# limanling/clip-event

Measured on AMD Instinct MI355X. Metric: image-text pairs/sec/GPU, ViT-B/32 224px x 77-tok, global-batch contrastive, higher is better.
Workload: dtype bf16; 1 GPU; ViT-B/32 224px x 77-tok, bf16 operands, per-GPU batch 256, K=1, InfoNCE only, full train step (fwd+bwd+clip_grad_norm+Adam), random-init weights; global_batch=256, parallelism=dp1, captions=SOT + U[8,75] random ids + EOT, zero-padded to 77 (SURVEY 8(d) c2), text_rows=live tokens SOT..EOT only: 54.8% of B*77 rows (identical results, see DESIGN.md), fresh_captions_every_step=True, alignment=False, cu_hog=0, nt_pgrid=256, full=False

## Files before the change

clip_event_amd/csrc/gemm.hip:

```cpp
#include <stdlib.h>

#include <map>
#include <mutex>
#include <type_traits>

#include "common.hpp"
#include "nt_plan.hpp"
#include "tn_plan.hpp"
#include "../../include/clip_event_hip.h"

#ifndef CE_DIAG_TN3
#define CE_DIAG_TN3 0
#endif

namespace {

constexpr int NT_BM = 128, NT_BN = 128, NT_BK = 64;
constexpr int NT_STAGE_BYTES = (NT_BM + NT_BN) * NT_BK * 2;
constexpr int NT_LDS_BYTES = 2 * NT_STAGE_BYTES;

#include "gemm_common.hpp"

template <int EPI>
__global__ __launch_bounds__(256, 2) void gemm_nt_kernel(NTArgs p) {
// ... 1224 lines not shown
        const int cur = mt & 1;
        if (mt + 1 < nmt) issue_loads(mt + 1);
        const char* st = smem + cur * TN_STAGE_BYTES;
#pragma unroll
        for (int s = 0; s < 4; ++s) {
            bf16x8 pf[2], qf[2];
#pragma unroll
            for (int t = 0; t < 2; ++t) {
                pf[t] = tr_frag(st, tp_base + s * 16 * TN_ROW + t * 64);
                qf[t] = tr_frag(st, tq_base + s * 16 * TN_ROW + t * 64);
            }
#pragma unroll
            for (int nt = 0; nt < 2; ++nt)
#pragma unroll
                for (int kt = 0; kt < 2; ++kt)
                    acc[nt][kt] = __builtin_amdgcn_mfma_f32_32x32x16_bf16(pf[nt], qf[kt], acc[nt][kt], 0, 0, 0);
        }
        if (mt + 1 < nmt) write_stage(cur ^ 1);
        __syncthreads();
    }

    const int ek = k0 + wk * 64 + (lane & 31);
    const int en = n0 + wn * 64 + 4 * (lane >> 5);
#pragma unroll
    for (int nt = 0; nt < 2; ++nt)
#pragma unroll
        for (int kt = 0; kt < 2; ++kt) {
            const int k = ek + kt * 32;
            if (k >= p.Kk) continue;
#pragma unroll
            for (int r = 0; r < 16; ++r) {
                const int n = en + nt * 32 + (r & 3) + 8 * (r >> 2);
                if (n < p.Nn) atomicAdd(p.out + (long)n * p.ldo + k, acc[nt][kt][r]);
            }
        }
}

constexpr int T2_TILE_BYTES = TN_BM * 256;
constexpr int T2_STAGE_BYTES = 2 * T2_TILE_BYTES;
constexpr int T2_LDS_BYTES = 2 * T2_STAGE_BYTES;

__device__ __forceinline__ bf16x8 tr_frag2(const char* p) {
    typedef __attribute__((address_space(3))) s16x4 lds_s16x4;
    s16x4 lo = __builtin_amdgcn_ds_read_tr16_b64_v4i16((lds_s16x4*)(p));
    s16x4 hi = __builtin_amdgcn_ds_read_tr16_b64_v4i16((lds_s16x4*)(p + 4 * 256));
    typedef __attribute__((ext_vector_type(8))) short s16x8;
    s16x8 v = {lo[0], lo[1], lo[2], lo[3], hi[0], hi[1], hi[2], hi[3]};
    return __builtin_bit_cast(bf16x8, v);
}

struct TNGroup {
    int count, splits, m_per_split, M, depth;
    int overwrite = 0;
    int tile_end[CE_TN_MAX_GROUP];
    TNArgs prob[CE_TN_MAX_GROUP];
};

__global__ __launch_bounds__(256, 2) void gemm_tn2_kernel(TNGroup grp) {
    extern __shared__ __attribute__((aligned(16))) char smem[];
    const int tid = threadIdx.x;
    const int lane = tid & 63;
    const int wave = __builtin_amdgcn_readfirstlane(tid >> 6);
    const int wn = wave >> 1, wk = wave & 1;

    const int m_tiles = (grp.M + TN_BM - 1) / TN_BM;
    const int mps = grp.m_per_split / TN_BM;
    const int s_r = lane >> 4;
    const int s_chunk = (lane & 15) ^ (s_r << 2);
    const int g = lane >> 4, li = lane & 15;
    const int t_row = 8 * (g >> 1) + (li >> 2);
    const int t_sw = (li >> 2) << 2;
    const int t_cb = 2 * (g & 1) + ((li & 3) >> 1);
    int offP[2], offQ[2];
#pragma unroll
    for (int t = 0; t < 2; ++t) {
        offP[t] = t_row * 256 + (((wn * 8 + t * 4 + t_cb) ^ t_sw) << 4) + (li & 1) * 8;
        offQ[t] = T2_TILE_BYTES + t_row * 256 + (((wk * 8 + t * 4 + t_cb) ^ t_sw) << 4) + (li & 1) * 8;
    }

    {
        const int lb = xcd_remap(blockIdx.x, gridDim.x);
        int tile = lb / grp.splits;
        const int mt0 = (lb - tile * grp.splits) * mps;
        const int mt1 = min(m_tiles, mt0 + mps);
        if (mt0 >= mt1) return;
        int pi = 0;
        while (pi + 1 < grp.count && tile >= grp.tile_end[pi]) ++pi;
        if (pi > 0) tile -= grp.tile_end[pi - 1];
        const TNArgs& p = grp.prob[pi];
        int tn, tk;
        {
            constexpr int BNB = 4, BKB = 4;
            const int br = tile / (BNB * p.tiles_k);
            const int r0 = br * BNB, rows_b = min(BNB, p.tiles_n - r0);
            const int t1 = tile - br * BNB * p.tiles_k;
            const int bc = t1 / (rows_b * BKB);
            const int c0 = bc * BKB, cols_b = min(BKB, p.tiles_k - c0);
            const int t2 = t1 - bc * rows_b * BKB;
            tn = r0 + t2 / cols_b;
            tk = c0 + t2 % cols_b;
        }
        const int n0 = tn * TN_BN, k0 = tk * TN_BK;
        const int ms = mt0 * TN_BM;
        const int rows = min(grp.M, mt1 * TN_BM) - ms;
        const long ldp = p.ldp, ldq = p.ldq;

        const u32x4 rP = make_rsrc_words(p.P + (long)ms * ldp, (uint32_t)((long)rows * ldp * 2));
        const u32x4 rQ = make_rsrc_words(p.Q + (long)ms * ldq, (uint32_t)((long)rows * ldq * 2));
        uint32_t vP[4], vQ[4];
// ... 17 lines not shown
        };

        f32x16 acc[2][2];
#pragma unroll
        for (int r = 0; r < 16; ++r) {
            acc[0][0][r] = 0.f; acc[0][1][r] = 0.f; acc[1][0][r] = 0.f; acc[1][1][r] = 0.f;
        }

        const int nmt = mt1 - mt0;
        stage(0, 0);
        asm volatile("s_waitcnt vmcnt(0)" ::: "memory");
        __syncthreads();
        for (int mt = 0; mt < nmt; ++mt) {
            const int cur = mt & 1;
            if (mt + 1 < nmt) stage(cur ^ 1, mt + 1);
            const char* st = smem + cur * T2_STAGE_BYTES;
#pragma unroll
            for (int s = 0; s < 4; ++s) {
                bf16x8 pf[2], qf[2];
#pragma unroll
                for (int t = 0; t < 2; ++t) {
                    pf[t] = tr_frag2(st + offP[t] + s * 16 * 256);
                    qf[t] = tr_frag2(st + offQ[t] + s * 16 * 256);
                }
#pragma unroll
                for (int nt = 0; nt < 2; ++nt)
#pragma unroll
                    for (int kt = 0; kt < 2; ++kt)
                        acc[nt][kt] = __builtin_amdgcn_mfma_f32_32x32x16_bf16(pf[nt], qf[kt], acc[nt][kt], 0, 0, 0);
            }
            asm volatile("s_waitcnt vmcnt(0)" ::: "memory");
            __syncthreads();
        }

        const int ek = k0 + wk * 64 + (lane & 31);
        const int en = n0 + wn * 64 + 4 * (lane >> 5);
        constexpr bool sole = false;
#pragma unroll
        for (int nt = 0; nt < 2; ++nt)
#pragma unroll
            for (int kt = 0; kt < 2; ++kt) {
                const int k = ek + kt * 32;
                if (k >= p.Kk) continue;
#pragma unroll
                for (int r = 0; r < 16; ++r) {
                    const int n = en + nt * 32 + (r & 3) + 8 * (r >> 2);
                    if (n < p.Nn) {
                        float* o = p.out + (long)n * p.ldo + k;
                        if (sole) *o += acc[nt][kt][r];
                        else atomicAdd(o, acc[nt][kt][r]);
                    }
                }
            }
    }
}

template <int T3_ROWS, int T3_STAGES>
__global__ __launch_bounds__(1024, 4) void gemm_tn3_kernel(TNGroup grp) {
    constexpr int T3_IMG_BYTES = T3_ROWS * 256;
    constexpr int T3_STAGE_BYTES = 4 * T3_IMG_BYTES;
    constexpr int KSTEPS = T3_ROWS / 16;
    constexpr int DPW = T3_ROWS / 16;
    extern __shared__ __attribute__((aligned(16))) char smem[];
    const int tid = threadIdx.x;
    const int lane = tid & 63;
    const int wave = __builtin_amdgcn_readfirstlane(tid >> 6);
    const int wn = wave >> 2, wk = wave & 3;

    const int m_tiles = (grp.M + TN_BM - 1) / TN_BM;
    const int mps = grp.m_per_split / TN_BM;
    const int s_r = lane >> 4;
    const int s_chunk = (lane & 15) ^ (s_r << 2);
    const int g = lane >> 4, li = lane & 15;
    const int t_row = 8 * (g >> 1) + (li >> 2);
    const int t_sw = (li >> 2) << 2;
    const int t_cb = 2 * (g & 1) + ((li & 3) >> 1);
    int offP[2], offQ[2];
#pragma unroll
    for (int t = 0; t < 2; ++t) {
        offP[t] = (wn >> 1) * T3_IMG_BYTES + t_row * 256 + ((((wn & 1) * 8 + t * 4 + t_cb) ^ t_sw) << 4) + (li & 1) * 8;
        offQ[t] = (2 + (wk >> 1)) * T3_IMG_BYTES + t_row * 256 + ((((wk & 1) * 8 + t * 4 + t_cb) ^ t_sw) << 4) + (li & 1) * 8;
    }

    const int lb = xcd_remap(blockIdx.x, gridDim.x);
    int tile = lb / grp.splits;
    const int mt0 = (lb - tile * grp.splits) * mps;
    const int mt1 = min(m_tiles, mt0 + mps);
    if (mt0 >= mt1) return;
    int pi = 0;
    while (pi + 1 < grp.count && tile >= grp.tile_end[pi]) ++pi;
    if (pi > 0) tile -= grp.tile_end[pi - 1];
    const TNArgs& p = grp.prob[pi];
    int tn, tk;
    {
        constexpr int BNB = 2, BKB = 2;
        const int br = tile / (BNB * p.tiles_k);
        const int r0 = br * BNB, rows_b = min(BNB, p.tiles_n - r0);
        const int t1 = tile - br * BNB * p.tiles_k;
        const int bc = t1 / (rows_b * BKB);
        const int c0 = bc * BKB, cols_b = min(BKB, p.tiles_k - c0);
        const int t2 = t1 - bc * rows_b * BKB;
        tn = r0 + t2 / cols_b;
        tk = c0 + t2 % cols_b;
    }
    const int n0 = tn * 256, k0 = tk * 256;
    const int ms = mt0 * TN_BM;
// ... 24 lines not shown
    for (int r = 0; r < 16; ++r) {
        acc[0][0][r] = 0.f; acc[0][1][r] = 0.f; acc[1][0][r] = 0.f; acc[1][1][r] = 0.f;
    }

    const int nst = (rows + T3_ROWS - 1) / T3_ROWS;
    const int D = min(grp.depth, T3_STAGES - 1);
    stage(0, 0);
    if (nst > 1 && D > 1) stage(1, 1);
    if (nst > 2 && D > 2) stage(2, 2);
    int slot = 0;
    for (int i = 0; i < nst; ++i) {
        const int later = min(nst - 1 - i, D - 1);
        if (later == 2) asm volatile("s_waitcnt vmcnt(%0)" ::"n"(2 * DPW) : "memory");
        else if (later == 1) asm volatile("s_waitcnt vmcnt(%0)" ::"n"(DPW) : "memory");
        else asm volatile("s_waitcnt vmcnt(0)" ::: "memory");
        __builtin_amdgcn_s_barrier();
        if (i + D < nst) {
            int sl = slot + D;
            if (sl >= T3_STAGES) sl -= T3_STAGES;
            stage(sl, i + D);
        }
        const char* st = smem + slot * T3_STAGE_BYTES;
        slot = slot + 1 == T3_STAGES ? 0 : slot + 1;
#pragma unroll
        for (int s = 0; s < KSTEPS; ++s) {
            bf16x8 pf[2], qf[2];
#pragma unroll
            for (int t = 0; t < 2; ++t) {
                pf[t] = tr_frag2(st + offP[t] + s * 16 * 256);
                qf[t] = tr_frag2(st + offQ[t] + s * 16 * 256);
            }
#pragma unroll
            for (int nt = 0; nt < 2; ++nt)
#pragma unroll
                for (int kt = 0; kt < 2; ++kt)
                    acc[nt][kt] = __builtin_amdgcn_mfma_f32_32x32x16_bf16(pf[nt], qf[kt], acc[nt][kt], 0, 0, 0);
        }
    }

    const int ek = k0 + wk * 64 + (lane & 31);
    const int en = n0 + wn * 64 + 4 * (lane >> 5);
#pragma unroll
    for (int nt = 0; nt < 2; ++nt)
#pragma unroll
        for (int kt = 0; kt < 2; ++kt) {
            const int k = ek + kt * 32;
#pragma unroll
            for (int r = 0; r < 16; ++r) {
                const int n = en + nt * 32 + (r & 3) + 8 * (r >> 2);
                if (grp.overwrite) __builtin_nontemporal_store(acc[nt][kt][r], p.out + (long)n * p.ldo + k);
                else atomicAdd(p.out + (long)n * p.ldo + k, acc[nt][kt][r]);
            }
        }
}

template <int T3_ROWS, int T3_STAGES>
__global__ __launch_bounds__(768, 3) void gemm_tn3lw_kernel(TNGroup grp) {
    constexpr int T3_IMG_BYTES = T3_ROWS * 256;
    constexpr int T3_STAGE_BYTES = 4 * T3_IMG_BYTES;
    constexpr int KSTEPS = T3_ROWS / 16;
    constexpr int DPL = T3_ROWS / 4;
    extern __shared__ __attribute__((aligned(16))) char smem[];
    const int tid = threadIdx.x;
    const int lane = tid & 63;
    const int wave = __builtin_amdgcn_readfirstlane(tid >> 6);
    const int wn = (wave >> 2) & 1, wk = wave & 3;

    const int m_tiles = (grp.M + TN_BM - 1) / TN_BM;
    const int mps = grp.m_per_split / TN_BM;
    const int s_r = lane >> 4;
    const int s_chunk = (lane & 15) ^ (s_r << 2);
    const int g = lane >> 4, li = lane & 15;
    const int t_row = 8 * (g >> 1) + (li >> 2);
    const int t_sw = (li >> 2) << 2;
    const int t_cb = 2 * (g & 1) + ((li & 3) >> 1);
    int offP[4], offQ[2];
#pragma unroll
    for (int t = 0; t < 4; ++t)
        offP[t] = wn * T3_IMG_BYTES + t_row * 256 + (((t * 4 + t_cb) ^ t_sw) << 4) + (li & 1) * 8;
#pragma unroll
    for (int t = 0; t < 2; ++t)
        offQ[t] = (2 + (wk >> 1)) * T3_IMG_BYTES + t_row * 256 + ((((wk & 1) * 8 + t * 4 + t_cb) ^ t_sw) << 4) + (li & 1) * 8;

    const int lb = xcd_remap(blockIdx.x, gridDim.x);
    int tile = lb / grp.splits;
    const int mt0 = (lb - tile * grp.splits) * mps;
    const int mt1 = min(m_tiles, mt0 + mps);
    if (mt0 >= mt1) return;
    int pi = 0;
    while (pi + 1 < grp.count && tile >= grp.tile_end[pi]) ++pi;
    if (pi > 0) tile -= grp.tile_end[pi - 1];
    const TNArgs& p = grp.prob[pi];
    int tn, tk;
    {
        constexpr int BNB = 2, BKB = 2;
        const int br = tile / (BNB * p.tiles_k);
        const int r0 = br * BNB, rows_b = min(BNB, p.tiles_n - r0);
        const int t1 = tile - br * BNB * p.tiles_k;
        const int bc = t1 / (rows_b * BKB);
        const int c0 = bc * BKB, cols_b = min(BKB, p.tiles_k - c0);
        const int t2 = t1 - bc * rows_b * BKB;
        tn = r0 + t2 / cols_b;
        tk = c0 + t2 % cols_b;
    }
    const int n0 = tn * 256, k0 = tk * 256;
    const int ms = mt0 * TN_BM;
// ... 21 lines not shown
#endif
                dma16_bounds(rsrc, d + j * 1024, vo0 + j * vstep + mb);
            }
        };
        stage(0, 0);
        if (nst > 1 && D > 1) stage(1, 1);
        if (nst > 2 && D > 2) stage(2, 2);
        int slot = 0;
        for (int i = 0; i < nst; ++i) {
            const int later = min(nst - 1 - i, D - 1);
            if (later == 2) asm volatile("s_waitcnt vmcnt(%0)" ::"n"(2 * DPL) : "memory");
            else if (later == 1) asm volatile("s_waitcnt vmcnt(%0)" ::"n"(DPL) : "memory");
            else asm volatile("s_waitcnt vmcnt(0)" ::: "memory");
            __builtin_amdgcn_s_barrier();
            if (i + D < nst) {
                int sl = slot + D;
                if (sl >= T3_STAGES) sl -= T3_STAGES;
                stage(sl, i + D);
            }
            slot = slot + 1 == T3_STAGES ? 0 : slot + 1;
        }
        return;
    }

    f32x16 acc[4][2];
#pragma unroll
    for (int nt = 0; nt < 4; ++nt)
#pragma unroll
        for (int r = 0; r < 16; ++r) {
            acc[nt][0][r] = 0.f; acc[nt][1][r] = 0.f;
        }
    int slot = 0;
    for (int i = 0; i < nst; ++i) {
        __builtin_amdgcn_s_barrier();
        const char* st = smem + slot * T3_STAGE_BYTES;
        slot = slot + 1 == T3_STAGES ? 0 : slot + 1;
#pragma unroll
        for (int s = 0; s < KSTEPS; ++s) {
            bf16x8 qf[2];
#pragma unroll
            for (int t = 0; t < 2; ++t) qf[t] = tr_frag2(st + offQ[t] + s * 16 * 256);
#pragma unroll
            for (int nt = 0; nt < 4; ++nt) {
                const bf16x8 pf = tr_frag2(st + offP[nt] + s * 16 * 256);
#pragma unroll
                for (int kt = 0; kt < 2; ++kt)
                    acc[nt][kt] = __builtin_amdgcn_mfma_f32_32x32x16_bf16(pf, qf[kt], acc[nt][kt], 0, 0, 0);
            }
        }
    }

    const int ek = k0 + wk * 64 + (lane & 31);
    const int en = n0 + wn * 128 + 4 * (lane >> 5);
#pragma unroll
    for (int nt = 0; nt < 4; ++nt)
#pragma unroll
        for (int kt = 0; kt < 2; ++kt) {
            const int k = ek + kt * 32;
#pragma unroll
            for (int r = 0; r < 16; ++r) {
                const int n = en + nt * 32 + (r & 3) + 8 * (r >> 2);
#if CE_DIAG_TN3 == 1
                if (acc[nt][kt][r] == 12345.678f)
#endif
                if (grp.overwrite) __builtin_nontemporal_store(acc[nt][kt][r], p.out + (long)n * p.ldo + k);
                else atomicAdd(p.out + (long)n * p.ldo + k, acc[nt][kt][r]);
            }
        }
}

__global__ void probe_mfma16_kernel(const bf16x8* a, const bf16x8* b, f32x4* out) {
    f32x4 c = {0.f, 0.f, 0.f, 0.f};
    c = __builtin_amdgcn_mfma_f32_16x16x32_bf16(a[threadIdx.x], b[threadIdx.x], c, 0, 0, 0);
    out[threadIdx.x] = c;
}
__global__ void probe_mfma32_kernel(const bf16x8* a, const bf16x8* b, f32x16* out) {
    f32x16 c;
#pragma unroll
    for (int r = 0; r < 16; ++r) c[r] = 0.f;
    c = __builtin_amdgcn_mfma_f32_32x32x16_bf16(a[threadIdx.x], b[threadIdx.x], c, 0, 0, 0);
    out[threadIdx.x] = c;
}
__global__ void probe_tr16_kernel(const uint16_t* image, int n_elems, const int* byte_off, s16x4* out) {
    extern __shared__ __attribute__((aligned(16))) char smem[];
    uint16_t* l = reinterpret_cast<uint16_t*>(smem);
    for (int i = threadIdx.x; i < n_elems; i += 64) l[i] = image[i];
    __syncthreads();
    typedef __attribute__((address_space(3))) s16x4 lds_s16x4;
    out[threadIdx.x] = __builtin_amdgcn_ds_read_tr16_b64_v4i16((lds_s16x4*)(smem + byte_off[threadIdx.x]));
}

static_assert(NT_PLAN_LDS[NT_NT128] == NT_LDS_BYTES && NT_PLAN_LDS[NT_NT256x2] == N2H_LDS_BYTES && NT_PLAN_LDS[NT_NT256x4] == N2_LDS_BYTES &&
              NT_PLAN_LDS[NT_NT32] == N3_LDS_BYTES && NT_PLAN_LDS[NT_NT160_RING] == N4_LDS_BYTES && NT_PLAN_LDS[NT_LW] == N4_LDS_BYTES &&
              NT_PLAN_LDS[NT_PERSIST] == N4P_LDS_BYTES && NT_PLAN_LDS[NT_SKINNY] == SK_LDS_BYTES &&
              NT_PLAN_BLOCK[NT_LW] == 64 * (8 + N4_LOADERS), "nt_plan.hpp is out of step with the kernels");

int env_int(const char* name, int otherwise) {
    const char* e = getenv(name);
    return e ? atoi(e) : otherwise;
}
NTKnobs knobs_from_env() {
    NTKnobs k;
    k.cus = env_int("CE_GEMM_CUS", 256);
    k.dynamic = env_int("CE_NT_DYNAMIC", 0);
    k.env_chunk = env_int("CE_NT_CHUNK", 0);
    k.env_pgrid = env_int("CE_NT_PGRID", 0);
// ... 175 lines not shown
        case CE_EPI_BIAS_F32:
            CE_CHECK_ARG(bias, "ce_gemm_nt: bias epilogue without bias");
            return launch_nt<CE_EPI_BIAS_F32, 0>(a, s);
        case CE_EPI_BIAS_RESID_F32:
            CE_CHECK_ARG(bias && resid && ldr >= N && ldr % 4 == 0, "ce_gemm_nt: residual epilogue needs bias+resid");
            return launch_nt<CE_EPI_BIAS_RESID_F32, 0>(a, s);
        case CE_EPI_BIAS_RESID_F16:
            CE_CHECK_ARG(bias && resid && ldr >= N && ldr % 8 == 0 && ldo % 8 == 0, "ce_gemm_nt: fp16 residual epilogue needs bias+resid, ldr/ldo multiples of 8");
            return launch_nt<CE_EPI_BIAS_RESID_F16, 0>(a, s);
        case CE_EPI_BIAS_GELU:
            CE_CHECK_ARG(bias && out2 && ldo2 >= N && ldo2 % 4 == 0, "ce_gemm_nt: gelu epilogue needs bias+out2");
            return launch_nt<CE_EPI_BIAS_GELU, 0>(a, s);
        case CE_EPI_BIAS_QGELU_BF16:
            CE_CHECK_ARG(bias, "ce_gemm_nt: QuickGELU epilogue without bias");
            return launch_nt<CE_EPI_BIAS_QGELU_BF16, 0>(a, s);
        case CE_EPI_GELUGRAD_BF16:
            CE_CHECK_ARG(aux && ldaux >= N && ldaux % 4 == 0, "ce_gemm_nt: gelu-grad epilogue needs aux");
            return launch_nt<CE_EPI_GELUGRAD_BF16, 0>(a, s);
        default: CE_CHECK_ARG(false, "ce_gemm_nt: unknown epilogue %d", epilogue);
    }
    return 0;
}

extern "C" int ce_gemm_tn(const void* P, long ldp, const void* Q, long ldq, int M, int Nn, int Kk, float* out,
                          long ldo, int splits, void* stream) {
    return ce_gemm_tn_bias(P, ldp, Q, ldq, M, Nn, Kk, out, ldo, nullptr, splits, stream);
}

extern "C" int ce_gemm_tn_bias(const void* P, long ldp, const void* Q, long ldq, int M, int Nn, int Kk, float* out,
                               long ldo, float* bias_grad, int splits, void* stream) {
    const void* Ps[1] = {P};
    const void* Qs[1] = {Q};
    float* outs[1] = {out};
    int rc = ce_gemm_tn_grouped(1, Ps, &ldp, Qs, &ldq, M, &Nn, &Kk, outs, &ldo, splits, stream);
    if (rc != 0) return rc;
    if (bias_grad) return ce_colsum_bf16(P, ldp, bias_grad, M, Nn, stream);
    return 0;
}

extern "C" int ce_gemm_tn_grouped(int count, const void* const* P, const long* ldp, const void* const* Q,
                                  const long* ldq, int M, const int* Nn, const int* Kk, float* const* out,
                                  const long* ldo, int splits, void* stream) {
    return ce_gemm_tn_grouped_ex(count, P, ldp, Q, ldq, M, Nn, Kk, out, ldo, splits, 0, stream);
}

static_assert(TN_PLAN_BM == TN_BM && TN_PLAN_LDS_V1 == TN_LDS_BYTES && TN_PLAN_LDS_128 == T2_LDS_BYTES &&
              tn_plan_lds_256(48, 3) == 3 * 48 * 1024 && tn_plan_lds_256(32, 4) == 4 * 32 * 1024 && TN_PLAN_BLOCK[TN_V1] == 256 &&
              TN_PLAN_BLOCK[TN_V2] == 256 && TN_PLAN_BLOCK[TN_V3] == 1024 && TN_PLAN_BLOCK[TN_V3LW] == 768,
              "tn_plan.hpp is out of step with the kernels");

extern "C" int ce_gemm_tn_grouped_ex(int count, const void* const* P, const long* ldp, const void* const* Q,
                                     const long* ldq, int M, const int* Nn, const int* Kk, float* const* out,
                                     const long* ldo, int splits, int overwrite, void* stream) {
    CE_CHECK_ARG(count >= 1 && count <= CE_TN_MAX_GROUP && M > 0, "ce_gemm_tn_grouped: 1..%d problems, M > 0", CE_TN_MAX_GROUP);
    hipStream_t s = (hipStream_t)stream;
    TNGroup g;
    g.count = count;
    g.M = M;
    double flops = 0.0, bytes = 0.0;
    long ldmax = 0;
    for (int i = 0; i < count; ++i) {
        CE_CHECK_ARG(Nn[i] > 0 && Kk[i] > 0, "ce_gemm_tn: empty problem");
        CE_CHECK_ARG(Nn[i] % 8 == 0 && Kk[i] % 8 == 0 && ldp[i] % 8 == 0 && ldq[i] % 8 == 0,
                     "ce_gemm_tn: Nn,Kk,ldp,ldq must be multiples of 8");
        CE_CHECK_ARG(ldp[i] >= Nn[i] && ldq[i] >= Kk[i] && ldo[i] >= Kk[i], "ce_gemm_tn: leading dimension smaller than the row");
        TNArgs& a = g.prob[i];
        a.P = (const bf16_t*)P[i]; a.ldp = ldp[i]; a.Q = (const bf16_t*)Q[i]; a.ldq = ldq[i];
        a.out = out[i]; a.ldo = ldo[i]; a.M = M; a.Nn = Nn[i]; a.Kk = Kk[i];
        flops += 2.0 * M * Nn[i] * Kk[i];
        bytes += 2.0 * ((double)M * Nn[i] + (double)M * Kk[i]) + 8.0 * Nn[i] * Kk[i];
        if (ldp[i] > ldmax) ldmax = ldp[i];
        if (ldq[i] > ldmax) ldmax = ldq[i];
    }
    CE_CHECK_ARG((long)M * ldmax * 2 < (1L << 32), "ce_gemm_tn: operand exceeds 4 GiB");

    const TNPlan p = tn_plan(M, count, Nn, Kk, splits, overwrite != 0, tn_process_knobs());
    g.splits = p.splits; g.m_per_split = p.m_per_split; g.depth = p.depth; g.overwrite = p.kernel_overwrites;
    for (int i = 0; i < CE_TN_MAX_GROUP; ++i) g.tile_end[i] = p.tile_end[i];
    for (int i = 0; i < count; ++i) {
        TNArgs& a = g.prob[i];
        a.tiles_n = p.tiles_n[i]; a.tiles_k = p.tiles_k[i]; a.splits = p.splits; a.m_per_split = p.m_per_split;
    }
    if (p.zero_fill_first)
        for (int i = 0; i < count; ++i)
            if (hipMemset2DAsync(out[i], (size_t)ldo[i] * 4, 0, (size_t)Kk[i] * 4, (size_t)Nn[i], s) != hipSuccess) {
                ce_set_error("ce_gemm_tn_grouped: zero-fill of output %d failed", i);
                return -5;
            }

    constexpr auto key = [](int form, int rows) { return 64 * form + rows; };
#define CE_TN_CASE(FORM, ROWS, ...)                                                      \
    case key(FORM, ROWS): {                                                              \
        CeProfScope prof(p.prof_class, flops, bytes, s);                                 \
        launch_kernel<__VA_ARGS__>(p.workgroups, p.block, p.lds_bytes, g, s);            \
    } break
    switch (key(p.form, p.rows)) {
        case key(TN_V1, 64):
            for (int i = 0; i < count; ++i) {
                const TNArgs& a = g.prob[i];
                CeProfScope prof(p.prof_class, 2.0 * M * a.Nn * a.Kk, 0.0, s);
                launch_kernel<gemm_tn_kernel>(a.tiles_n * a.tiles_k * a.splits, p.block, p.lds_bytes, a, s);
            }
            break;
        CE_TN_CASE(TN_V2, 64, gemm_tn2_kernel);
        CE_TN_CASE(TN_V3, 32, gemm_tn3_kernel<32, 4>);
        CE_TN_CASE(TN_V3, 48, gemm_tn3_kernel<48, 3>);
        CE_TN_CASE(TN_V3LW, 48, gemm_tn3lw_kernel<48, 3>);
        CE_TN_CASE(TN_V3LW, 32, gemm_tn3lw_kernel<32, 4>);
        default: CE_CHECK_ARG(false, "ce_gemm_tn_grouped: no kernel of form %d with %d-row stages", (int)p.form, p.rows);
    }
#undef CE_TN_CASE
    CE_LAUNCH_CHECK();
    return 0;
}

extern "C" int ce_gemm_tn_plan(int count, const int* Nn, const int* Kk, int M, int splits, int overwrite, const ce_tn_knobs* knobs,
                               ce_tn_plan* out) {
    CE_CHECK_ARG(out && Nn && Kk && count >= 1 && count <= CE_TN_MAX_GROUP && M > 0,
                 "ce_gemm_tn_plan: 1..%d problems, M > 0 and a result struct", CE_TN_MAX_GROUP);
    for (int i = 0; i < count; ++i) CE_CHECK_ARG(Nn[i] > 0 && Kk[i] > 0, "ce_gemm_tn_plan: empty problem %d", i);
    *out = tn_plan(M, count, Nn, Kk, splits, overwrite != 0, knobs ? TNKnobs(*knobs) : tn_process_knobs());
    return 0;
}

extern "C" int ce_probe_mfma(int shape, const void* a_frags, const void* b_frags, float* out, void* stream) {
    if (shape == 16)
        hipLaunchKernelGGL(probe_mfma16_kernel, dim3(1), dim3(64), 0, (hipStream_t)stream, (const bf16x8*)a_frags,
                           (const bf16x8*)b_frags, (f32x4*)out);
    else if (shape == 32)
        hipLaunchKernelGGL(probe_mfma32_kernel, dim3(1), dim3(64), 0, (hipStream_t)stream, (const bf16x8*)a_frags,
                           (const bf16x8*)b_frags, (f32x16*)out);
    else
        CE_CHECK_ARG(false, "ce_probe_mfma: shape must be 16 or 32");
    CE_LAUNCH_CHECK();
    return 0;
}

extern "C" int ce_probe_tr16(const void* image, int n_elems, const int* byte_off, void* out, void* stream) {
    CE_CHECK_ARG(n_elems > 0 && n_elems <= 16384, "ce_probe_tr16: image must hold 1..16384 elements");
    hipLaunchKernelGGL(probe_tr16_kernel, dim3(1), dim3(64), n_elems * 2, (hipStream_t)stream, (const uint16_t*)image,
                       n_elems, byte_off, (s16x4*)out);
    CE_LAUNCH_CHECK();
    return 0;
}
```

clip_event_amd/csrc/optim.hip:

```cpp
#include <stdlib.h>

#include "common.hpp"
#include "../../include/clip_event_hip.h"

#ifndef CE_ADAM_NT
#define CE_ADAM_NT 2
#endif
#if CE_ADAM_NT >= 1
#define CE_ADAM_ST(val, ptr) __builtin_nontemporal_store(val, ptr)
#else
#define CE_ADAM_ST(val, ptr) (*(ptr) = (val))
#endif
#if CE_ADAM_NT >= 2
#define CE_ADAM_LD(ptr) __builtin_nontemporal_load(ptr)
#else
#define CE_ADAM_LD(ptr) (*(ptr))
#endif

namespace {

__global__ __launch_bounds__(256) void sumsq_kernel(const float* __restrict__ g, long n, float* __restrict__ out) {
    __shared__ float red[4];
    float s = 0.f;
    const long stride = gridDim.x * 1024L;
// ... 261 lines not shown
}
template <class Rule>
__device__ __forceinline__ void store_state(float* const (&st)[2], long at, const f32x4 (&sv)[kSlots<Rule>]) {
#pragma unroll
    for (int k = 0; k < Rule::NS; ++k) CE_ADAM_ST(sv[k], reinterpret_cast<f32x4*>(st[k] + at));
}
__device__ __forceinline__ u32x2 pack_bf4(const f32x4& v) { return u32x2{pack_bf2(v[0], v[1]), pack_bf2(v[2], v[3])}; }

template <class Rule, bool EMA>
__global__ __launch_bounds__(256) void optim_flat_kernel(float* __restrict__ p, const float* __restrict__ g, float* __restrict__ s0,
                                                         float* __restrict__ s1, bf16_t* __restrict__ p16, long n,
                                                         typename Rule::Args a, float* __restrict__ ema, float ema_rate) {
    const Rule rule(a, 0);
    float* const st[2] = {s0, s1};
    const long stride = gridDim.x * 2048L;
    for (long i0 = blockIdx.x * 2048L + threadIdx.x * 4; i0 < n; i0 += stride) {
        const long i1 = i0 + 1024;
        if (i1 + 3 < n) {
            f32x4 pv[2], gv[2], sv[2][kSlots<Rule>] = {}, ev[2] = {};
#pragma unroll
            for (int u = 0; u < 2; ++u) load_chunk<Rule, EMA>(p, g, st, ema, u ? i1 : i0, pv[u], gv[u], sv[u], ev[u]);
#pragma unroll
            for (int u = 0; u < 2; ++u) {
                const long i = u ? i1 : i0;
                elem4(rule, pv[u], gv[u], sv[u]);
                CE_ADAM_ST(pv[u], reinterpret_cast<f32x4*>(p + i));
                if (p16) *reinterpret_cast<u32x2*>(p16 + i) = pack_bf4(pv[u]);
                store_state<Rule>(st, i, sv[u]);
                update_ema<EMA>(ema, i, ev[u], pv[u], ema_rate);
            }
        } else {
            for (int u = 0; u < 2; ++u) {
                const long ib = u ? i1 : i0;
                for (long k = ib; k < n && k < ib + 4; ++k) {
                    float pk = p[k], sk[kSlots<Rule>] = {};
#pragma unroll
                    for (int q = 0; q < Rule::NS; ++q) sk[q] = st[q][k];
                    rule.elem(pk, g[k], sk);
                    p[k] = pk;
#pragma unroll
                    for (int q = 0; q < Rule::NS; ++q) st[q][k] = sk[q];
                    if (p16) p16[k] = f2bf(pk);
                    if constexpr (EMA) {
                        float ek = ema[k];
                        ema_elem(ek, pk, ema_rate);
                        ema[k] = ek;
                    }
                }
            }
        }
    }
}

__global__ __launch_bounds__(256) void zero_segments_kernel(float* __restrict__ base, const long* __restrict__ table) {
    const long lo = table[2 * blockIdx.x], hi = table[2 * blockIdx.x + 1];
    for (long i = lo + threadIdx.x * 4; i < hi; i += 1024)
        __builtin_nontemporal_store(f32x4{0.f, 0.f, 0.f, 0.f}, reinterpret_cast<f32x4*>(base + i));
}

struct tile_at {
    ce_transpose_job job;
    int r0, c0;
};
__device__ __forceinline__ tile_at find_tile(const ce_transpose_job* __restrict__ jobs, int njobs) {
    int j = 0;
    const int b = blockIdx.x;
    while (j + 1 < njobs && b >= jobs[j + 1].tile_start) ++j;
    const ce_transpose_job job = jobs[j];
    const int t = b - job.tile_start;
    const int tiles_c = (job.cols + 63) / 64;
    return {job, (t / tiles_c) * 64, (t % tiles_c) * 64};
}

template <bool NT>
__device__ __forceinline__ void store_tile_transposed(const bf16_t (&tile)[64][66], const tile_at& t) {
    bf16_t* dst = reinterpret_cast<bf16_t*>(t.job.dst);
#pragma unroll
    for (int k = 0; k < 2; ++k) {
        const int idx = threadIdx.x + k * 256;
        const int c = idx >> 3, ch = idx & 7;
        if (t.c0 + c < t.job.cols && t.r0 + ch * 8 < t.job.rows) {
            uint32_t w[4];
#pragma unroll
            for (int e = 0; e < 4; ++e)
                w[e] = (uint32_t)tile[ch * 8 + 2 * e][c] | ((uint32_t)tile[ch * 8 + 2 * e + 1][c] << 16);
            const u32x4 v = {w[0], w[1], w[2], w[3]};
            u32x4* out = reinterpret_cast<u32x4*>(dst + (long)(t.c0 + c) * t.job.rows + t.r0 + ch * 8);
            if (NT) __builtin_nontemporal_store(v, out);
            else *out = v;
        }
    }
}

__global__ __launch_bounds__(256) void multi_transpose_kernel(const ce_transpose_job* __restrict__ jobs, int njobs) {
    __shared__ bf16_t tile[64][66];
    const tile_at t = find_tile(jobs, njobs);
    const ce_transpose_job& job = t.job;
    const int r0 = t.r0, c0 = t.c0;
    const bf16_t* src = reinterpret_cast<const bf16_t*>(job.src);
    bf16_t* dst = reinterpret_cast<bf16_t*>(job.dst);
    const bool wide = (job.rows % 8 == 0) && (job.cols % 8 == 0) &&
                      ((reinterpret_cast<size_t>(src) | reinterpret_cast<size_t>(dst)) % 16 == 0);
    if (wide) {
#pragma unroll
        for (int k = 0; k < 2; ++k) {
            const int idx = threadIdx.x + k * 256;
            const int r = idx >> 3, ch = idx & 7;
// ... 142 lines not shown
    const long blocks = (n + 2047) / 2048;
    return (unsigned)(blocks > cap ? cap : blocks);
}
template <class Rule>
void launch_flat(float* p, const float* g, float* s0, float* s1, void* p_bf16, long n, const typename Rule::Args& a, void* stream,
                 float* ema = nullptr, float ema_rate = 0.f) {
    if (ema)
        hipLaunchKernelGGL((optim_flat_kernel<Rule, true>), dim3(flat_blocks(n)), dim3(256), 0, (hipStream_t)stream, p, g, s0, s1,
                           (bf16_t*)p_bf16, n, a, ema, ema_rate);
    else
        hipLaunchKernelGGL((optim_flat_kernel<Rule, false>), dim3(flat_blocks(n)), dim3(256), 0, (hipStream_t)stream, p, g, s0, s1,
                           (bf16_t*)p_bf16, n, a, ema, 0.f);
}

template <class Rule>
void launch_tiles(float* p, const float* g, float* s0, float* s1, void* p_bf16, const ce_transpose_job* jobs_device, int njobs,
                  int total_tiles, const long* segments_device, int nsegments, const typename Rule::Args& a, void* stream,
                  float* ema = nullptr, float ema_rate = 0.f) {
    const hipStream_t s = (hipStream_t)stream;
    if (jobs_device && njobs > 0 && total_tiles > 0) {
        if (ema)
            hipLaunchKernelGGL((optim_tiles_kernel<Rule, true>), dim3((unsigned)total_tiles), dim3(256), 0, s, p, g, s0, s1,
                               (bf16_t*)p_bf16, jobs_device, njobs, a, ema, ema_rate);
        else
            hipLaunchKernelGGL((optim_tiles_kernel<Rule, false>), dim3((unsigned)total_tiles), dim3(256), 0, s, p, g, s0, s1,
                               (bf16_t*)p_bf16, jobs_device, njobs, a, ema, 0.f);
    }
    if (segments_device && nsegments > 0) {
        if (ema)
            hipLaunchKernelGGL((optim_segments_kernel<Rule, true>), dim3((unsigned)nsegments), dim3(256), 0, s, p, g, s0, s1,
                               (bf16_t*)p_bf16, segments_device, a, ema, ema_rate);
        else
            hipLaunchKernelGGL((optim_segments_kernel<Rule, false>), dim3((unsigned)nsegments), dim3(256), 0, s, p, g, s0, s1,
                               (bf16_t*)p_bf16, segments_device, a, ema, 0.f);
    }
}

int ema_check(const char* who, const float* ema, float ema_rate) {
    CE_CHECK_ARG(ema, "%s: ema is NULL", who);
    CE_CHECK_ARG(ema_rate > 0.f && ema_rate <= 1.f, "%s: ema_rate %g is outside (0, 1]", who, (double)ema_rate);
    return 0;
}

}

extern "C" int ce_multi_transpose_bf16(const ce_transpose_job* jobs_device, int njobs, int total_tiles, void* stream) {
    CE_CHECK_ARG(jobs_device && njobs > 0 && total_tiles > 0, "ce_multi_transpose_bf16: empty");
    hipLaunchKernelGGL(multi_transpose_kernel, dim3(total_tiles), dim3(256), 0, (hipStream_t)stream, jobs_device, njobs);
    CE_LAUNCH_CHECK();
    return 0;
}

extern "C" int ce_zero_segments(float* base, const long* table_device, int nchunks, void* stream) {
    CE_CHECK_ARG(base && table_device && nchunks > 0, "ce_zero_segments: empty");
    hipLaunchKernelGGL(zero_segments_kernel, dim3(nchunks), dim3(256), 0, (hipStream_t)stream, base, table_device);
    CE_LAUNCH_CHECK();
    return 0;
}

extern "C" int ce_sumsq(const float* g, long n, float* out, void* stream) {
    CE_CHECK_ARG(n > 0, "ce_sumsq: empty");
    long blocks = (n + 1023) / 1024;
    if (blocks > 2048) blocks = 2048;
    hipLaunchKernelGGL(sumsq_kernel, dim3((unsigned)blocks), dim3(256), 0, (hipStream_t)stream, g, n, out);
    CE_LAUNCH_CHECK();
    return 0;
}


namespace {

int adam_step(const char* who, float* p, const float* g, float* m, float* v, void* p_bf16, long n, const float* sumsq, float max_norm,
              float lr, float beta1, float beta2, float eps, float weight_decay, int step, float* ema, float ema_rate, void* stream) {
    CE_CHECK_ARG(n > 0 && step >= 1, "%s: need n>0 and step>=1", who);
    launch_flat<AdamRule>(p, g, m, v, p_bf16, n, adam_args(sumsq, max_norm, lr, beta1, beta2, eps, weight_decay, step), stream, ema,
                          ema_rate);
    CE_LAUNCH_CHECK();
    return 0;
}

int adam_step_tiles(const char* who, float* p, const float* g, float* m, float* v, void* p_bf16, const ce_transpose_job* jobs_device,
                    int njobs, int total_tiles, const long* segments_device, int nsegments, const float* sumsq, float max_norm, float lr,
                    float beta1, float beta2, float eps, float weight_decay, int step, float* ema, float ema_rate, void* stream) {
    CE_CHECK_ARG(p && g && m && v && p_bf16 && step >= 1, "%s: null buffer or step < 1", who);
    CE_CHECK_ARG((jobs_device && njobs > 0 && total_tiles > 0) || (segments_device && nsegments > 0), "%s: nothing to update", who);
    launch_tiles<AdamRule>(p, g, m, v, p_bf16, jobs_device, njobs, total_tiles, segments_device, nsegments,
                           adam_args(sumsq, max_norm, lr, beta1, beta2, eps, weight_decay, step), stream, ema, ema_rate);
    CE_LAUNCH_CHECK();
    return 0;
}

int sgd_step(const char* who, float* p, const float* g, float* buf, void* p_bf16, long n, const float* sumsq, float max_norm, float lr,
             float momentum, float dampening, float weight_decay, int nesterov, int first_step, float* ema, float ema_rate,
             void* stream) {
    CE_CHECK_ARG(n > 0, "%s: need n>0", who);
    if (int rc = sgd_check(who, buf, momentum, dampening, nesterov)) return rc;
    CE_CHECK_ARG(p && g, "%s: null buffer", who);
    const sgd_args a = {sumsq, max_norm, lr, momentum, 1.0f - dampening, weight_decay, first_step != 0, nesterov != 0};
    if (momentum > 0.f) launch_flat<SgdRule<true>>(p, g, buf, nullptr, p_bf16, n, a, stream, ema, ema_rate);
    else launch_flat<SgdRule<false>>(p, g, nullptr, nullptr, p_bf16, n, a, stream, ema, ema_rate);
    CE_LAUNCH_CHECK();
    return 0;
}

int sgd_step_tiles(const char* who, float* p, const float* g, float* buf, void* p_bf16, const ce_transpose_job* jobs_device, int njobs,
                   int total_tiles, const long* segments_device, int nsegments, const float* sumsq, float max_norm, float lr,
                   float momentum, float dampening, float weight_decay, int nesterov, int first_step, float* ema, float ema_rate,
                   void* stream) {
    if (int rc = sgd_check(who, buf, momentum, dampening, nesterov)) return rc;
    CE_CHECK_ARG((jobs_device && njobs > 0 && total_tiles > 0) || (segments_device && nsegments > 0), "%s: nothing to update", who);
    CE_CHECK_ARG(p && g && p_bf16, "%s: null buffer", who);
    const sgd_args a = {sumsq, max_norm, lr, momentum, 1.0f - dampening, weight_decay, first_step != 0, nesterov != 0};
    if (momentum > 0.f)
        launch_tiles<SgdRule<true>>(p, g, buf, nullptr, p_bf16, jobs_device, njobs, total_tiles, segments_device, nsegments, a, stream,
                                    ema, ema_rate);
    else
// ... 103 lines not shown
                                float* ema, float ema_rate, void* stream) {
    if (int rc = ema_check("ce_adam_step_ema", ema, ema_rate)) return rc;
    return adam_step("ce_adam_step_ema", p, g, m, v, p_bf16, n, sumsq, max_norm, lr, beta1, beta2, eps, weight_decay, step, ema,
                     ema_rate, stream);
}

extern "C" int ce_adam_step_tiles(float* p, const float* g, float* m, float* v, void* p_bf16, const ce_transpose_job* jobs_device,
                                  int njobs, int total_tiles, const long* segments_device, int nsegments, const float* sumsq,
                                  float max_norm, float lr, float beta1, float beta2, float eps, float weight_decay, int step,
                                  void* stream) {
    return adam_step_tiles("ce_adam_step_tiles", p, g, m, v, p_bf16, jobs_device, njobs, total_tiles, segments_device, nsegments, sumsq,
                           max_norm, lr, beta1, beta2, eps, weight_decay, step, nullptr, 0.f, stream);
}
extern "C" int ce_adam_step_tiles_ema(float* p, const float* g, float* m, float* v, void* p_bf16, const ce_transpose_job* jobs_device,
                                      int njobs, int total_tiles, const long* segments_device, int nsegments, const float* sumsq,
                                      float max_norm, float lr, float beta1, float beta2, float eps, float weight_decay, int step,
                                      float* ema, float ema_rate, void* stream) {
    if (int rc = ema_check("ce_adam_step_tiles_ema", ema, ema_rate)) return rc;
    return adam_step_tiles("ce_adam_step_tiles_ema", p, g, m, v, p_bf16, jobs_device, njobs, total_tiles, segments_device, nsegments,
                           sumsq, max_norm, lr, beta1, beta2, eps, weight_decay, step, ema, ema_rate, stream);
}

extern "C" int ce_sgd_step(float* p, const float* g, float* buf, void* p_bf16, long n, const float* sumsq, float max_norm, float lr,
                           float momentum, float dampening, float weight_decay, int nesterov, int first_step, void* stream) {
    return sgd_step("ce_sgd_step", p, g, buf, p_bf16, n, sumsq, max_norm, lr, momentum, dampening, weight_decay, nesterov, first_step,
                    nullptr, 0.f, stream);
}
extern "C" int ce_sgd_step_ema(float* p, const float* g, float* buf, void* p_bf16, long n, const float* sumsq, float max_norm, float lr,
                               float momentum, float dampening, float weight_decay, int nesterov, int first_step, float* ema,
                               float ema_rate, void* stream) {
    if (int rc = ema_check("ce_sgd_step_ema", ema, ema_rate)) return rc;
    return sgd_step("ce_sgd_step_ema", p, g, buf, p_bf16, n, sumsq, max_norm, lr, momentum, dampening, weight_decay, nesterov,
                    first_step, ema, ema_rate, stream);
}

extern "C" int ce_sgd_step_tiles(float* p, const float* g, float* buf, void* p_bf16, const ce_transpose_job* jobs_device, int njobs,
                                 int total_tiles, const long* segments_device, int nsegments, const float* sumsq, float max_norm,
                                 float lr, float momentum, float dampening, float weight_decay, int nesterov, int first_step,
                                 void* stream) {
    return sgd_step_tiles("ce_sgd_step_tiles", p, g, buf, p_bf16, jobs_device, njobs, total_tiles, segments_device, nsegments, sumsq,
                          max_norm, lr, momentum, dampening, weight_decay, nesterov, first_step, nullptr, 0.f, stream);
}
extern "C" int ce_sgd_step_tiles_ema(float* p, const float* g, float* buf, void* p_bf16, const ce_transpose_job* jobs_device, int njobs,
                                     int total_tiles, const long* segments_device, int nsegments, const float* sumsq, float max_norm,
                                     float lr, float momentum, float dampening, float weight_decay, int nesterov, int first_step,
                                     float* ema, float ema_rate, void* stream) {
    if (int rc = ema_check("ce_sgd_step_tiles_ema", ema, ema_rate)) return rc;
    return sgd_step_tiles("ce_sgd_step_tiles_ema", p, g, buf, p_bf16, jobs_device, njobs, total_tiles, segments_device, nsegments, sumsq,
                          max_norm, lr, momentum, dampening, weight_decay, nesterov, first_step, ema, ema_rate, stream);
}

extern "C" int ce_sumsq_segments(const float* g, const long* table_device, int nchunks, float* out, void* stream) {
    CE_CHECK_ARG(g && table_device && out && nchunks > 0, "ce_sumsq_segments: empty");
    hipLaunchKernelGGL(sumsq_segments_kernel, dim3((unsigned)nchunks), dim3(256), 0, (hipStream_t)stream, g, table_device, out);
    CE_LAUNCH_CHECK();
    return 0;
}

extern "C" int ce_adam_step_groups(float* p, const float* g, float* m, float* v, void* p_bf16, const ce_transpose_job* jobs_device,
                                   int njobs, int total_tiles, const long* segments_device, int nsegments, const int* segment_group,
                                   const float* sumsq, float max_norm, const ce_optim_group* groups, int ngroups, float beta1,
                                   float beta2, float eps, int step, void* stream) {
    return adam_step_groups("ce_adam_step_groups", p, g, m, v, p_bf16, jobs_device, njobs, total_tiles, segments_device, nsegments,
                            segment_group, sumsq, max_norm, groups, ngroups, beta1, beta2, eps, step, nullptr, 0.f, stream);
}
extern "C" int ce_adam_step_groups_ema(float* p, const float* g, float* m, float* v, void* p_bf16, const ce_transpose_job* jobs_device,
                                       int njobs, int total_tiles, const long* segments_device, int nsegments, const int* segment_group,
                                       const float* sumsq, float max_norm, const ce_optim_group* groups, int ngroups, float beta1,
                                       float beta2, float eps, int step, float* ema, float ema_rate, void* stream) {
    if (int rc = ema_check("ce_adam_step_groups_ema", ema, ema_rate)) return rc;
    return adam_step_groups("ce_adam_step_groups_ema", p, g, m, v, p_bf16, jobs_device, njobs, total_tiles, segments_device, nsegments,
                            segment_group, sumsq, max_norm, groups, ngroups, beta1, beta2, eps, step, ema, ema_rate, stream);
}

extern "C" int ce_sgd_step_groups(float* p, const float* g, float* buf, void* p_bf16, const ce_transpose_job* jobs_device, int njobs,
                                  int total_tiles, const long* segments_device, int nsegments, const int* segment_group,
                                  const float* sumsq, float max_norm, const ce_optim_group* groups, int ngroups, float momentum,
                                  float dampening, int nesterov, int first_step, void* stream) {
    return sgd_step_groups("ce_sgd_step_groups", p, g, buf, p_bf16, jobs_device, njobs, total_tiles, segments_device, nsegments,
                           segment_group, sumsq, max_norm, groups, ngroups, momentum, dampening, nesterov, first_step, nullptr, 0.f,
                           stream);
}
extern "C" int ce_sgd_step_groups_ema(float* p, const float* g, float* buf, void* p_bf16, const ce_transpose_job* jobs_device, int njobs,
                                      int total_tiles, const long* segments_device, int nsegments, const int* segment_group,
                                      const float* sumsq, float max_norm, const ce_optim_group* groups, int ngroups, float momentum,
                                      float dampening, int nesterov, int first_step, float* ema, float ema_rate, void* stream) {
    if (int rc = ema_check("ce_sgd_step_groups_ema", ema, ema_rate)) return rc;
    return sgd_step_groups("ce_sgd_step_groups_ema", p, g, buf, p_bf16, jobs_device, njobs, total_tiles, segments_device, nsegments,
                           segment_group, sumsq, max_norm, groups, ngroups, momentum, dampening, nesterov, first_step, ema, ema_rate,
                           stream);
}

extern "C" int ce_lion_step(float* p, const float* g, float* m, void* p_bf16, long n, const float* sumsq, float max_norm, float lr,
                            float beta1, float beta2, float weight_decay, void* stream) {
    return lion_step("ce_lion_step", p, g, m, p_bf16, n, sumsq, max_norm, lr, beta1, beta2, weight_decay, nullptr, 0.f, stream);
}
extern "C" int ce_lion_step_ema(float* p, const float* g, float* m, void* p_bf16, long n, const float* sumsq, float max_norm, float lr,
                                float beta1, float beta2, float weight_decay, float* ema, float ema_rate, void* stream) {
    if (int rc = ema_check("ce_lion_step_ema", ema, ema_rate)) return rc;
    return lion_step("ce_lion_step_ema", p, g, m, p_bf16, n, sumsq, max_norm, lr, beta1, beta2, weight_decay, ema, ema_rate, stream);
}

extern "C" int ce_lion_step_tiles(float* p, const float* g, float* m, void* p_bf16, const ce_transpose_job* jobs_device, int njobs,
                                  int total_tiles, const long* segments_device, int nsegments, const float* sumsq, float max_norm,
                                  float lr, float beta1, float beta2, float weight_decay, void* stream) {
    return lion_step_tiles("ce_lion_step_tiles", p, g, m, p_bf16, jobs_device, njobs, total_tiles, segments_device, nsegments, sumsq,
// ... 36 lines not shown
```

clip_event_amd/csrc/tn_plan.cpp:

```cpp
#include "tn_plan.hpp"

#include <stdlib.h>

namespace {

inline int div_up(long a, long b) { return (int)((a + b - 1) / b); }

inline void set_splits(TNPlan& p, int M, int splits) {
    const int m_tiles = div_up(M, TN_PLAN_BM);
    if (splits > m_tiles) splits = m_tiles;
    if (splits < 1) splits = 1;
    p.m_per_split = div_up(m_tiles, splits) * TN_PLAN_BM;
    p.splits = div_up(M, p.m_per_split);
}

inline int env_int(const char* name, int otherwise) {
    const char* e = getenv(name);
    return e ? atoi(e) : otherwise;
}

}

TNKnobs tn_knobs_from_env() {
    TNKnobs k;
// ... 29 lines not shown
        p.lds_bytes = p.form == TN_V1 ? TN_PLAN_LDS_V1 : TN_PLAN_LDS_128;
        set_splits(p, M, splits_arg > 0 ? splits_arg : 512 / tiles);
        p.prof_class = CE_PROF_GEMM_TN2;
    } else {
        auto cost = [&](int sp) {
            const long wgs = (long)tiles * sp;
            const long rounds = (wgs + 255) / 256;
            const long tail = wgs - (rounds - 1) * 256;
            return rounds * (div_up(m_tiles, sp) * 1.7 + 3.0) + tail * (sp == 1 ? 0.105 : 0.20);
        };
        int sp = 1;
        if (splits_arg > 0) sp = splits_arg;
        else if (knobs.force_splits > 0) sp = knobs.force_splits;
        else {
            double best = cost(1);
            for (int c = 2; c <= 16 && c <= m_tiles && (long)tiles * c <= 256; ++c)
                if (cost(c) < best) { best = cost(c); sp = c; }
        }
        set_splits(p, M, sp);
        p.rows = knobs.rows == 32 ? 32 : 48;
        p.stages = p.rows == 48 ? 3 : 4;
        p.form = knobs.loader_waves ? TN_V3LW : TN_V3;
        p.lds_bytes = tn_plan_lds_256(p.rows, p.stages);
        p.kernel_overwrites = overwrite && p.splits == 1;
        p.prof_class = CE_PROF_GEMM_TN;
    }
    p.zero_fill_first = overwrite && !p.kernel_overwrites;
    p.block = TN_PLAN_BLOCK[p.form];
    p.workgroups = tiles * p.splits;
    return p;
}

int tn_group_cuts(int n_blocks, int width, int M, long extra_tiles, int force_group, int* sizes_out) {
    const int n = n_blocks;
    if (force_group > TN_GROUP_MAX_BLOCKS) force_group = TN_GROUP_MAX_BLOCKS;
    const long t = 12 * tn_problem_tiles(M, width, width);
    const long slots = tn_round_slots(M, width, width);
    long cost[TN_CUT_MAX_BLOCKS + 1];
    int take[TN_CUT_MAX_BLOCKS + 1];
    cost[0] = 0;
    for (int k = 1; k <= n; ++k) {
        cost[k] = -1;
        for (int g = 1; g <= TN_GROUP_MAX_BLOCKS && g <= k; ++g) {
            if (force_group >= 1 && g != force_group && g != k) continue;
            const long tiles = g * t + (k == n ? extra_tiles : 0);
            const long c = cost[k - g] + (tiles + slots - 1) / slots * 1000 + 1;
            if (cost[k] < 0 || c < cost[k]) { cost[k] = c; take[k] = g; }
        }
    }
    int groups = 0;
    for (int k = n; k > 0; k -= take[k]) sizes_out[groups++] = take[k];
    return groups;
}
```

clip_event_amd/csrc/tn_plan.hpp:

```cpp
#pragma once
#include "../../include/clip_event_hip.h"

enum TNForm {
    TN_V1 = 0,
    TN_V2 = 1,
    TN_V3 = 2,
    TN_V3LW = 3
};

constexpr int TN_PLAN_BLOCK[4] = {256, 256, 1024, 768};
constexpr int TN_PLAN_LDS_128 = 65536;
constexpr int TN_PLAN_LDS_V1 = 81920;
constexpr int tn_plan_lds_256(int rows, int stages) { return stages * rows * 1024; }

constexpr int TN_PLAN_BM = 64;
constexpr int TN_PLAN_MIN_M_256 = 2048;

constexpr bool tn_tiles_256(int M, int Nn, int Kk) { return M >= TN_PLAN_MIN_M_256 && Nn % 256 == 0 && Kk % 256 == 0; }
constexpr long tn_problem_tiles(int M, int Nn, int Kk) {
    return tn_tiles_256(M, Nn, Kk) ? (long)(Nn / 256) * (Kk / 256) : (long)((Nn + 127) / 128) * ((Kk + 127) / 128);
}
constexpr int tn_round_slots(int M, int Nn, int Kk) { return tn_tiles_256(M, Nn, Kk) ? 256 : 512; }

struct TNKnobs : ce_tn_knobs {
    constexpr TNKnobs() : ce_tn_knobs{3, 0, 3, 48, 1} {}
    constexpr TNKnobs(const ce_tn_knobs& k) : ce_tn_knobs(k) {}
};
TNKnobs tn_knobs_from_env();
const TNKnobs& tn_process_knobs();

using TNPlan = ce_tn_plan;

TNPlan tn_plan(int M, int count, const int* Nn, const int* Kk, int splits_arg, bool overwrite, const TNKnobs& knobs);

constexpr int TN_CUT_MAX_BLOCKS = 64;
constexpr int TN_GROUP_MAX_BLOCKS = 8;

int tn_group_cuts(int n_blocks, int width, int M, long extra_tiles, int force_group, int* sizes_out);
```

clip_event_amd/csrc/tower.cpp:

```cpp
#include <hip/hip_runtime.h>
#include <stdlib.h>

#include <map>
#include <mutex>

#include "common.hpp"
#include "tn_plan.hpp"
#include "../../include/clip_event_hip.h"

namespace {

constexpr int WG_MAX_BLOCKS = TN_GROUP_MAX_BLOCKS;
constexpr int WG_SETS = WG_MAX_BLOCKS + 1;
constexpr int LNP_RING = 8;

struct Carver {
    char* base;
    size_t off = 0;
    explicit Carver(void* b) : base(reinterpret_cast<char*>(b)) {}
    template <typename T>
    T* take(size_t n) {
        off = (off + 255) & ~size_t(255);
        T* p = base ? reinterpret_cast<T*>(base + off) : nullptr;
        off += n * sizeof(T);
        return p;
    }
};

struct BlockStash {
    void* x_mid;
    void* x_out;
    bf16_t *h1, *qkv, *o, *h2, *a, *g;
    float *mean1, *rstd1, *mean2, *rstd2, *lse;
};

struct Layout {
    static constexpr int MAX_LAYERS = 64;
    BlockStash blk[MAX_LAYERS];
    bf16_t *dxb[WG_SETS], *dxb2[WG_SETS], *da[WG_SETS], *dqkv[WG_SETS];
    bf16_t *dh, *d_o;
    uint8_t* q8;
    float* q8s;
    float *xs_in, *xs_mid, *dxs_mid, *means, *rstds;
    bf16_t *os, *h2s, *as, *gs, *dxbs, *dxb2s, *das, *dhs, *dos;
    float* lnp[LNP_RING][2];
    size_t bytes;
};

void carve(const ce_tower_desc* d, int batch, size_t rows, void* ws, Layout& L) {
    Carver c(ws);
    const size_t M = rows, w = d->width;
    const size_t esz = d->stream16 ? 2 : 4;
    for (int l = 0; l < d->layers; ++l) {
        BlockStash& s = L.blk[l];
        s.x_mid = c.take<char>(M * w * esz);
        s.x_out = (l + 1 < d->layers) ? c.take<char>(M * w * esz) : nullptr;
        s.h1 = c.take<bf16_t>(M * w);
        s.qkv = c.take<bf16_t>(M * 3 * w);
        s.o = c.take<bf16_t>(M * w);
        s.h2 = c.take<bf16_t>(M * w);
        s.a = c.take<bf16_t>(M * 4 * w);
        s.g = c.take<bf16_t>(M * 4 * w);
        s.mean1 = c.take<float>(M);
        s.rstd1 = c.take<float>(M);
        s.mean2 = c.take<float>(M);
        s.rstd2 = c.take<float>(M);
        s.lse = c.take<float>((size_t)batch * d->heads * d->tokens);
    }
    for (int q = 0; q < WG_SETS; ++q) {
        L.dxb[q] = c.take<bf16_t>(M * w);
        L.dxb2[q] = c.take<bf16_t>(M * w);
        L.da[q] = c.take<bf16_t>(M * 4 * w);
        L.dqkv[q] = c.take<bf16_t>(M * 3 * w);
    }
    L.dh = c.take<bf16_t>(M * w);
    L.d_o = c.take<bf16_t>(M * w);
    L.q8 = d->fp8 ? c.take<uint8_t>(M * 4 * w) : nullptr;
    L.q8s = d->fp8 ? c.take<float>(M) : nullptr;
    const size_t Bn = (size_t)batch;
    L.xs_in = c.take<float>(Bn * w); L.xs_mid = c.take<float>(Bn * w); L.dxs_mid = c.take<float>(Bn * w);
    L.means = c.take<float>(Bn); L.rstds = c.take<float>(Bn);
    L.os = c.take<bf16_t>(Bn * w); L.h2s = c.take<bf16_t>(Bn * w); L.as = c.take<bf16_t>(Bn * 4 * w); L.gs = c.take<bf16_t>(Bn * 4 * w);
    L.dxbs = c.take<bf16_t>(Bn * w); L.dxb2s = c.take<bf16_t>(Bn * w); L.das = c.take<bf16_t>(Bn * 4 * w);
    L.dhs = c.take<bf16_t>(Bn * w); L.dos = c.take<bf16_t>(Bn * w);
    const size_t lnp_floats = (size_t)ce_layernorm_bwd_blocks((int)M, (int)w) * 3 * w;
    for (int l = 0; l < LNP_RING; ++l) {
        L.lnp[l][0] = l < d->layers ? c.take<float>(lnp_floats) : nullptr;
        L.lnp[l][1] = l < d->layers ? c.take<float>(lnp_floats) : nullptr;
    }
    L.bytes = (c.off + 255) & ~size_t(255);
}

void carve_infer(const ce_tower_desc* d, int batch, size_t rows, void* ws, Layout& L) {
    Carver c(ws);
    const size_t M = rows, w = d->width;
    const size_t esz = d->stream16 ? 2 : 4;
    L = Layout{};
    BlockStash s{};
    s.x_mid = c.take<char>(M * w * esz);
    s.x_out = c.take<char>(M * w * esz);
    s.h1 = s.h2 = c.take<bf16_t>(M * w);
    s.qkv = c.take<bf16_t>(M * 3 * w);
    s.o = c.take<bf16_t>(M * w);
    s.a = nullptr;
    s.g = c.take<bf16_t>(M * 4 * w);
    s.mean1 = s.mean2 = c.take<float>(M);
    s.rstd1 = s.rstd2 = c.take<float>(M);
    s.lse = c.take<float>((size_t)batch * d->heads * d->tokens);
    for (int l = 0; l < d->layers; ++l) L.blk[l] = s;
    L.blk[d->layers - 1].x_out = nullptr;
    L.q8 = d->fp8 ? c.take<uint8_t>(M * 4 * w) : nullptr;
    L.q8s = d->fp8 ? c.take<float>(M) : nullptr;
    const size_t Bn = (size_t)batch;
    L.xs_in = c.take<float>(Bn * w); L.xs_mid = c.take<float>(Bn * w);
    L.means = c.take<float>(Bn); L.rstds = c.take<float>(Bn);
    L.os = c.take<bf16_t>(Bn * w); L.h2s = c.take<bf16_t>(Bn * w); L.gs = c.take<bf16_t>(Bn * 4 * w);
    L.bytes = (c.off + 255) & ~size_t(255);
}

int check_rows(const ce_tower_desc* d, int batch, int rows, const int* cu) {
    CE_CHECK_ARG(rows > 0 && (long)rows <= (long)batch * d->tokens, "tower: rows=%d outside 1..batch*tokens", rows);
    CE_CHECK_ARG(cu || rows == batch * d->tokens, "tower: a dense batch has batch*tokens rows (got %d)", rows);
    return 0;
}

int check_desc(const ce_tower_desc* d, int batch) {
    CE_CHECK_ARG(d && d->blocks, "tower: null descriptor");
    CE_CHECK_ARG(d->layers > 0 && d->layers <= Layout::MAX_LAYERS, "tower: layers=%d out of range", d->layers);
    CE_CHECK_ARG(d->width == d->heads * 64, "tower: width %d != heads %d * 64", d->width, d->heads);
    CE_CHECK_ARG(d->tokens > 0 && d->tokens <= 4096, "tower: tokens=%d unsupported (1..4096)", d->tokens);
    CE_CHECK_ARG(batch > 0, "tower: empty batch");
    CE_CHECK_ARG(d->stream16 == 0 || d->stream16 == 1, "tower: stream16=%d (0: fp32 residual stream, 1: fp16)", d->stream16);
    return 0;
}

#define TRY(call)            \
    do {                     \
        int rc__ = (call);   \
        if (rc__ != 0) return rc__; \
    } while (0)

// ... 69 lines not shown
extern "C" int ce_tower_forward(const ce_tower_desc* d, int batch, int rows, const int* cu_seqlens, const void* x0,
                                void* workspace, void* x_out, const int* sel_rows, void* stream) {
    TRY(check_desc(d, batch));
    TRY(check_rows(d, batch, rows, cu_seqlens));
    CE_CHECK_ARG(x0 && workspace && x_out, "ce_tower_forward: null buffer");
    Layout L;
    carve(d, batch, rows, workspace, L);
    return forward_run(d, batch, rows, cu_seqlens, x0, L, x_out, sel_rows, false, stream);
}

extern "C" size_t ce_tower_infer_workspace_bytes(const ce_tower_desc* d, int batch) {
    if (check_desc(d, batch) != 0) return 0;
    Layout L;
    carve_infer(d, batch, (size_t)batch * d->tokens, nullptr, L);
    return L.bytes;
}

extern "C" int ce_tower_forward_infer(const ce_tower_desc* d, int batch, int rows, const int* cu_seqlens, const void* x0,
                                      void* workspace, void* x_out, const int* sel_rows, void* stream) {
    TRY(check_desc(d, batch));
    TRY(check_rows(d, batch, rows, cu_seqlens));
    CE_CHECK_ARG(x0 && workspace && x_out, "ce_tower_forward_infer: null buffer");
    Layout L;
    carve_infer(d, batch, rows, workspace, L);
    return forward_run(d, batch, rows, cu_seqlens, x0, L, x_out, sel_rows, true, stream);
}

extern "C" int ce_tower_backward(const ce_tower_desc* d, int batch, int rows, const int* cu_seqlens, const void* x0,
                                 void* workspace, void* dx, const int* sel_rows, const float* dx_sel, void* stream) {
    return ce_tower_backward_range(d, batch, rows, cu_seqlens, x0, workspace, dx, sel_rows, dx_sel,
                                   d ? d->layers - 1 : 0, 0, stream);
}

extern "C" int ce_tower_backward_range(const ce_tower_desc* d, int batch, int rows, const int* cu_seqlens,
                                       const void* x0, void* workspace, void* dx, const int* sel_rows,
                                       const float* dx_sel, int layer_hi, int layer_lo, void* stream) {
    TRY(check_desc(d, batch));
    TRY(check_rows(d, batch, rows, cu_seqlens));
    CE_CHECK_ARG(x0 && workspace && dx, "ce_tower_backward: null buffer");
    CE_CHECK_ARG(layer_lo >= 0 && layer_lo <= layer_hi && layer_hi < d->layers, "ce_tower_backward_range: layers %d..%d outside 0..%d",
                 layer_hi, layer_lo, d->layers - 1);
    Layout L;
    carve(d, batch, rows, workspace, L);
    const int M = rows, w = d->width;
    const bool b8 = (d->fp8 & 2) != 0;
    const int ST = d->stream16 ? CE_T_F16 : CE_T_F32;
    const void* q8_of = nullptr;
    const bool lnq = b8 && w % 128 == 0 && w <= 4096;
    const float* GS = d->stream16 ? d->grad_scale : nullptr;
    CE_CHECK_ARG(!d->stream16 || GS, "ce_tower_backward: stream16 needs ce_tower_desc.grad_scale (device pointer)");
    const long esz = d->stream16 ? 2 : 4;
    const int last = d->layers - 1;
    static const int ln_fold = getenv("CE_LN_FOLD") ? atoi(getenv("CE_LN_FOLD")) : 1;
    ce_ln_fold_job fold_jobs[2 * LNP_RING];
    int n_fold = 0;
    int fold_rc = 0;
    const int ln_blocks = ce_layernorm_bwd_blocks(M, w);
    auto ln_bwd = [&](const void* dy, const void* xin, const float* mean, const float* rstd, const float* gamma, void* dxb, float* dgw, float* dgb,
                      float* dxs, void* q8, float* partial) -> int {
        if (!ln_fold)
            return ce_layernorm_bwd_q8(dy, CE_T_BF16, w, xin, ST, w, nullptr, mean, rstd, gamma, dx, ST, dx, ST, w, dxb, w, dgw, dgb, dxs, GS, M, w, q8, w,
                                       L.q8s, stream);
        fold_jobs[n_fold++] = ce_ln_fold_job{partial, dgw, dgb, dxs, ln_blocks, w};
        const int rc = ce_layernorm_bwd_partials(dy, CE_T_BF16, w, xin, ST, w, nullptr, mean, rstd, gamma, dx, ST, dx, ST, w, dxb, w, dxs ? 1 : 0, GS, M, w, q8, w,
                                                 L.q8s, partial, stream);
        if (rc == 0 && n_fold == 2 * LNP_RING) {
            fold_rc = ce_layernorm_fold(fold_jobs, n_fold, stream);
            n_fold = 0;
            return fold_rc;
        }
        return rc;
    };
    static const int force_group = getenv("CE_WGRAD_GROUP") ? atoi(getenv("CE_WGRAD_GROUP")) : 0;
    bool cut_after[Layout::MAX_LAYERS] = {};
    auto plan_cuts = [&](int hi, int lo, long extra_tiles) {
        static_assert(Layout::MAX_LAYERS <= TN_CUT_MAX_BLOCKS, "tn_group_cuts takes fewer blocks than a tower has");
        int sizes[Layout::MAX_LAYERS];
        const int groups = tn_group_cuts(hi - lo + 1, w, M, extra_tiles, force_group, sizes);
        int l = hi;
        for (int i = 0; i < groups; ++i) {
            l -= sizes[i];
            cut_after[l + 1] = true;
        }
    };
    struct Pending {
        const void* P[CE_TN_MAX_GROUP]; long ldp[CE_TN_MAX_GROUP];
        const void* Q[CE_TN_MAX_GROUP]; long ldq[CE_TN_MAX_GROUP];
        int Nn[CE_TN_MAX_GROUP], Kk[CE_TN_MAX_GROUP];
        float* out[CE_TN_MAX_GROUP]; long ldo[CE_TN_MAX_GROUP];
        int count = 0, blocks = 0;
    } pend;
    auto queue = [&](const void* P, long ldp, const void* Q, long ldq, int Nn, int Kk, float* out, long ldo) {
        const int i = pend.count++;
        pend.P[i] = P; pend.ldp[i] = ldp; pend.Q[i] = Q; pend.ldq[i] = ldq;
        pend.Nn[i] = Nn; pend.Kk[i] = Kk; pend.out[i] = out; pend.ldo[i] = ldo;
    };
    auto flush = [&]() -> int {
        if (pend.count == 0) return 0;
        const int rc = ce_gemm_tn_grouped_ex(pend.count, pend.P, pend.ldp, pend.Q, pend.ldq, M, pend.Nn, pend.Kk, pend.out,
                                             pend.ldo, 0, d->wgrad_overwrite, stream);
        pend.count = 0;
        pend.blocks = 0;
        return rc;
    };
    int top = layer_hi;
    if (layer_hi < last) {
    } else if (sel_rows) {
        CE_CHECK_ARG(dx_sel, "ce_tower_backward: pruned mode needs dx_sel");
        const int l = top, Bn = batch, q = l % WG_SETS;
        const ce_block_params& p = d->blocks[l];
        BlockStash& s = L.blk[l];
        const void* x_in = (l == 0) ? x0 : L.blk[l - 1].x_out;
        TRY(ce_cast_bf16(dx_sel, L.dxbs, (long)Bn * w, stream));
        TRY(linear(b8, L, q8_of, L.dxbs, w, p.wt_proj, p.wt8_proj, p.st8_proj, Bn, 4 * w, w, CE_EPI_GELUGRAD_BF16, nullptr, nullptr, 0, L.das, 4 * w, nullptr,
                       0, L.as, 4 * w, stream));
        TRY(ce_colsum_bf16(L.dxbs, w, p.g_b_proj, Bn, w, stream));
        TRY(linear(b8, L, q8_of, L.das, 4 * w, p.wt_fc, p.wt8_fc, p.st8_fc, Bn, w, 4 * w, CE_EPI_BF16, nullptr, nullptr, 0, L.dhs, w, nullptr, 0,
                       nullptr, 0, stream));
        TRY(ce_colsum_bf16(L.das, 4 * w, p.g_b_fc, Bn, 4 * w, stream));
        TRY(ce_layernorm_bwd_t(L.dhs, CE_T_BF16, w, L.xs_mid, ST, w, nullptr, L.means, L.rstds, p.ln2_w, dx_sel, CE_T_F32, L.dxs_mid,
                               ST, w, L.dxb2s, w, p.g_ln2_w, p.g_ln2_b, p.g_b_out, GS, Bn, w, stream));
        TRY(linear(b8, L, q8_of, L.dxb2s, w, p.wt_out, p.wt8_out, p.st8_out, Bn, w, w, CE_EPI_BF16, nullptr, nullptr, 0, L.dos, w, nullptr, 0, nullptr, 0,
                       stream));
        TRY(ce_scatter_rows_zero(L.dos, w * 2L, L.d_o, w * 2L, sel_rows, Bn, M, w * 2, stream));
        TRY(ce_attention_bwd(s.qkv, 3 * w, s.o, w, L.d_o, w, s.lse, L.dqkv[q], 3 * w, p.g_b_qkv, cu_seqlens, batch, d->tokens, d->heads,
                             d->causal, stream));
        {
            const void* P[3] = {L.dxbs, L.das, L.dxb2s};
            const long ldp[3] = {w, 4L * w, w};
            const void* Q[3] = {L.gs, L.h2s, L.os};
            const long ldq[3] = {4L * w, w, w};
            const int Nn[3] = {w, 4 * w, w};
            const int Kk[3] = {4 * w, w, w};
            float* out[3] = {p.g_w_proj, p.g_w_fc, p.g_w_out};
            const long ldo[3] = {4L * w, w, w};
            TRY(ce_gemm_tn_grouped_ex(3, P, ldp, Q, ldq, Bn, Nn, Kk, out, ldo, 0, d->wgrad_overwrite, stream));
        }
        queue(L.dqkv[q], 3L * w, s.h1, w, 3 * w, w, p.g_w_qkv, w);
        TRY(linear(b8, L, q8_of, L.dqkv[q], 3 * w, p.wt_qkv, p.wt8_qkv, p.st8_qkv, M, w, 3 * w, CE_EPI_BF16, nullptr, nullptr, 0, L.dh, w, nullptr, 0,
                       nullptr, 0, stream));
        TRY(ce_scatter_rows_zero(L.dxs_mid, w * esz, dx, w * esz, sel_rows, Bn, M, (int)(w * esz), stream));
        TRY(ce_layernorm_bwd_t(L.dh, CE_T_BF16, w, x_in, ST, w, nullptr, s.mean1, s.rstd1, p.ln1_w, dx, ST, dx, ST, w,
                               L.dxb[(l + WG_SETS - 1) % WG_SETS], w, p.g_ln1_w, p.g_ln1_b,
                               (l > 0) ? d->blocks[l - 1].g_b_proj : nullptr, GS, M, w, stream));
        top = l - 1;
    } else {
        if (d->stream16) TRY(ce_cast_scaled(dx, ST, L.dxb[top % WG_SETS], CE_T_BF16, GS, 1, (long)M * w, stream));
        else TRY(ce_cast_bf16(reinterpret_cast<const float*>(dx), L.dxb[top % WG_SETS], (long)M * w, stream));
    }
    plan_cuts(top, layer_lo, pend.count > 0 ? 3 * tn_problem_tiles(M, w, w) : 0);
    for (int l = top; l >= layer_lo; --l) {
        const ce_block_params& p = d->blocks[l];
        BlockStash& s = L.blk[l];
        const int q = l % WG_SETS;
        bf16_t *dxb_a = L.dxb[q], *dxb_b = L.dxb2[q], *da = L.da[q], *dqkv = L.dqkv[q];
        const void* x_in = (l == 0) ? x0 : L.blk[l - 1].x_out;
        TRY(linear(b8, L, q8_of, dxb_a, w, p.wt_proj, p.wt8_proj, p.st8_proj, M, 4 * w, w, CE_EPI_GELUGRAD_BF16, nullptr, nullptr, 0, da, 4 * w, p.g_b_fc,
                       4 * w, s.a, 4 * w, stream));
        if (l == last) TRY(ce_colsum_bf16(dxb_a, w, p.g_b_proj, M, w, stream));
        TRY(linear(b8, L, q8_of, da, 4 * w, p.wt_fc, p.wt8_fc, p.st8_fc, M, w, 4 * w, CE_EPI_BF16, nullptr, nullptr, 0, L.dh, w, nullptr, 0,
                       nullptr, 0, stream));
        TRY(ln_bwd(L.dh, s.x_mid, s.mean2, s.rstd2, p.ln2_w, dxb_b, p.g_ln2_w, p.g_ln2_b, p.g_b_out, lnq ? L.q8 : nullptr, L.lnp[l % LNP_RING][1]));
        if (lnq) q8_of = dxb_b;
        TRY(linear(b8, L, q8_of, dxb_b, w, p.wt_out, p.wt8_out, p.st8_out, M, w, w, CE_EPI_BF16, nullptr, nullptr, 0, L.d_o, w, nullptr, 0, nullptr, 0,
                       stream));
        TRY(ce_attention_bwd(s.qkv, 3 * w, s.o, w, L.d_o, w, s.lse, dqkv, 3 * w, p.g_b_qkv, cu_seqlens, batch, d->tokens, d->heads,
                             d->causal, stream));
        queue(dxb_a, w, s.g, 4L * w, w, 4 * w, p.g_w_proj, 4L * w);
        queue(da, 4L * w, s.h2, w, 4 * w, w, p.g_w_fc, w);
        queue(dxb_b, w, s.o, w, w, w, p.g_w_out, w);
        queue(dqkv, 3L * w, s.h1, w, 3 * w, w, p.g_w_qkv, w);
        ++pend.blocks;
        if (cut_after[l] || pend.count + 4 > CE_TN_MAX_GROUP) TRY(flush());
        TRY(linear(b8, L, q8_of, dqkv, 3 * w, p.wt_qkv, p.wt8_qkv, p.st8_qkv, M, w, 3 * w, CE_EPI_BF16, nullptr, nullptr, 0, L.dh, w, nullptr, 0,
                       nullptr, 0, stream));
        TRY(ln_bwd(L.dh, x_in, s.mean1, s.rstd1, p.ln1_w, L.dxb[(l + WG_SETS - 1) % WG_SETS], p.g_ln1_w, p.g_ln1_b,
                   (l > 0) ? d->blocks[l - 1].g_b_proj : nullptr, (lnq && l > layer_lo) ? L.q8 : nullptr, L.lnp[l % LNP_RING][0]));
        if (lnq && l > layer_lo) q8_of = L.dxb[(l + WG_SETS - 1) % WG_SETS];
    }
    TRY(flush());
    if (n_fold > 0) TRY(ce_layernorm_fold(fold_jobs, n_fold, stream));
    return 0;
}

extern "C" int ce_tower_wgrad_cuts(int n_blocks, int width, int M, long extra_tiles, int force_group, int* sizes_out) {
    CE_CHECK_ARG(sizes_out && n_blocks >= 1 && n_blocks <= TN_CUT_MAX_BLOCKS && width > 0 && M > 0 && extra_tiles >= 0,
                 "ce_tower_wgrad_cuts: 1..%d blocks, width, M > 0, extra_tiles >= 0 and a result array", TN_CUT_MAX_BLOCKS);
    return tn_group_cuts(n_blocks, width, M, extra_tiles, force_group, sizes_out);
}
```

clip_event_amd/engine.py:

```python
from __future__ import annotations

import contextlib
import functools
import logging
import math
import operator
import os
import sys
from typing import Dict, Optional

import numpy as np
import torch

from . import distributed as D
from .functional import (attach_lengths, distill_losses, fused_contrastive_losses, fused_head_ok, logits_from_features,
                         sigmoid_contrastive_losses, small_contrastive_losses, small_head_ok, tokens_to_device)
from .losses import CriterionAlignment, CriterionContrastive, CriterionDistill


def _unwrap(model):
    return model.module if isinstance(model, D.DistributedDataParallel) else model


class Distillation:
# ... 301 lines not shown
                                               teacher=teacher)
        _sum_losses(loss_dict, check_finite).backward()
        for lo, hi, img_c, txt_c in (chunks if live else []):
            if len(live) == 2:
                with pinned(lo):
                    outs = model.encode_both(img_c, txt_c)
                grads = [fi.grad[lo:hi], ft.grad[lo * K:hi * K]]
            elif live[0] == "visual":
                with pinned(lo):
                    outs = [model.encode_image(img_c)]
                grads = [fi.grad[lo:hi]]
            else:
                outs, grads = [model.encode_text(txt_c)], [ft.grad[lo * K:hi * K]]
            torch.autograd.backward(list(outs), grads)
            del outs
    finally:
        model._lease_batch = None
    return loss_dict


def train_step(model, criterion, optimizer, image, text, labels_per_image, labels_per_text, index_pos,
               grad_sync: Optional[D.GradSync] = None, criterion_ot: Optional[CriterionAlignment] = None,
               object_vec=None, entitytxt_vec=None, object_num=None, entitytxt_num=None,
               check_finite: bool = False, train_arg=None, bboxs=None, bbox_desc_vec=None,
               bbox_label_vec=None, text_lengths=None, micro_batch: Optional[int] = None, distill: Optional[Distillation] = None,
               teacher_image=None, teacher_features=None) -> Dict[str, torch.Tensor]:
    wrapped = model
    model = _unwrap(model)
    chunked = micro_batch is not None and int(micro_batch) < int(image.shape[0])
    if chunked and (train_arg is not None or criterion_ot is not None):
        raise NotImplementedError("train_step(micro_batch=...) covers the plain contrastive step only: the region / alignment "
                                  "losses of train_arg / criterion_ot couple rows inside the towers' outputs; run that "
                                  "configuration without micro_batch")
    dev = next(model.parameters()).device
    _throttle(model)
    if text_lengths is not None:
        attach_lengths(text, text_lengths)
    text = tokens_to_device(text, dev)
    if entitytxt_vec is not None:
        entitytxt_vec = tokens_to_device(entitytxt_vec, dev)
    if grad_sync is None and wrapped is not model:
        grad_sync = wrapped.grad_sync
    teacher = None
    if distill is not None:
        distill.check_student(model)
        distill.check_optimizer(optimizer)
        if teacher_features is not None:
            teacher = (distill, teacher_features[0], teacher_features[1])
        elif not chunked:
            teacher = (distill,) + tuple(distill.encode(image, text, teacher_image))
    elif teacher_image is not None or teacher_features is not None:
        raise ValueError("teacher_image / teacher_features need distill=Distillation(...)")
    if hasattr(optimizer, "zero_grad_first_touch"):
        optimizer.zero_grad_first_touch()
    else:
        optimizer.zero_grad()
    want_align = model.alignment and criterion_ot is not None
    if chunked:
        loss_dict = micro_batched_backward(model, criterion, image, text, labels_per_image, labels_per_text, index_pos,
                                           int(micro_batch), grad_sync=grad_sync, check_finite=check_finite, distill=distill,
                                           teacher_image=teacher_image, teacher_features=teacher_features)
    elif (want_align or train_arg is not None) and os.environ.get("CE_MERGE_PASSES", "1") != "0":
        loss_dict = merged_step_losses(model, criterion, criterion_ot if want_align else None, image, text, labels_per_image,
                                       labels_per_text, index_pos, train_arg=train_arg, bboxs=bboxs, bbox_desc_vec=bbox_desc_vec,
                                       bbox_label_vec=bbox_label_vec, object_vec=object_vec, entitytxt_vec=entitytxt_vec,
                                       object_num=object_num, entitytxt_num=entitytxt_num, teacher=teacher)
    else:
        loss_dict = contrastive_step_losses(model, criterion, image, text, labels_per_image, labels_per_text, index_pos,
                                            train_arg=train_arg, bboxs=bboxs, bbox_desc_vec=bbox_desc_vec,
                                            bbox_label_vec=bbox_label_vec, teacher=teacher)
        if want_align:
            image_features, text_features = model.sim_entity(object_vec, entitytxt_vec)
            loss_dict.update(criterion_ot(text_features, image_features, entitytxt_num, object_num))
    if not chunked:
        _sum_losses(loss_dict, check_finite).backward()
    if check_finite and getattr(model, "stream16", False):
        sat_f, sat_g = model.stream16_saturation()
        if sat_f or sat_g:
            logging.error("fp16 stream saturated ({} forward, {} gradient slots), stopping training".format(sat_f, sat_g))
            sys.exit(1)
    if hasattr(model, "_settle_first_touch"):
        model._settle_first_touch()
    if grad_sync is not None:
        grad_sync.finish()
    optimizer.step()
    _mark_step_end(model)
    return loss_dict
```

clip_event_amd/functional.py:

```python
from __future__ import annotations

import ctypes
import os
import weakref

import numpy as np
import torch

from . import _lib as L
from . import ops
from ._lib import check, lib, ptr, stream


def _f32(t: torch.Tensor) -> torch.Tensor:
    return t if (t.dtype == torch.float32 and t.is_contiguous()) else t.contiguous().float()


def _tower_workspace(model, desc, batch: int, tag: str, infer: bool = False):
    from .model import _Lease
    fn = lib().ce_tower_infer_workspace_bytes if infer else lib().ce_tower_workspace_bytes
    hint = getattr(model, "_lease_batch", None)
    nbytes = fn(ctypes.byref(desc), max(batch, hint.get(tag, 0)) if hint else batch)
    if nbytes == 0:
        raise RuntimeError(fn.__name__ + ": " + lib().ce_last_error().decode())
    if infer:
        tag = tag + ".infer"
    buf = model._pool.take(tag, int(nbytes), model._flat.device)
    return _Lease(model._pool, tag, buf)


def _tower_forward_infer(model, desc, tag: str, batch: int, rows: int, cu, x0, x_out, sel):
    lease = _tower_workspace(model, desc, batch, tag, infer=True)
    check(lib().ce_tower_forward_infer(ctypes.byref(desc), batch, rows, ptr(cu), ptr(x0), ptr(lease.buf),
                                       ptr(x_out), ptr(sel), stream()), f"ce_tower_forward_infer({tag})")
    lease.release()


def _publish_to_main(ctx):
    ms = ctx.main_stream
    if ms is not None:
        cur = torch.cuda.current_stream()
        if cur != ms:
            ms.wait_stream(cur)


def _tower_backward(model, desc, tower: str, batch: int, rows: int, cu, x0, lease, dx, sel, dx_sel):
    cl, s = lib(), stream()
    layers = desc.layers
    stop = model.trainable_plan().stop_layer[tower]
    cuts = model.grad_sync.layer_cuts(tower, layers) if (model.grad_sync is not None and
                                                           hasattr(model.grad_sync, "layer_cuts")) else []
    cuts = [c for c in cuts if c > stop]
    owner = getattr(desc, "_owner", desc)
    cut = getattr(owner, "_cut", 0)
    if cut != stop:
        prefix = "visual.transformer." if tower == "visual" else "transformer."
        if 0 < cut < layers:
            desc.blocks[cut - 1].g_b_proj = model._gview(f"{prefix}resblocks.{cut - 1}.mlp.c_proj.bias").data_ptr()
        if 0 < stop < layers:
            desc.blocks[stop - 1].g_b_proj = None
        owner._cut = stop
    model.wait_transposes()
    pending = getattr(model, "_first_touch", None)
    desc.wgrad_overwrite = 1 if (pending and tower in pending) else 0
    if desc.wgrad_overwrite:
        pending.discard(tower)
    hi = layers - 1
    for lo in (list(cuts) + [stop] if stop < layers else []):
        check(cl.ce_tower_backward_range(ctypes.byref(desc), batch, rows, ptr(cu), ptr(x0), ptr(lease.buf), ptr(dx), ptr(sel),
                                         ptr(dx_sel), hi, lo, s), f"ce_tower_backward_range({tower})")
        if lo > stop:
            model.grad_sync(model, tower, upto_layer=lo)
        hi = lo - 1
    return stop


class TextPacking:
    __slots__ = ("rows", "cu", "src", "sel", "_keep")

    def __init__(self, rows, cu, src, sel, keep=None):
        self.rows, self.cu, self.src, self.sel, self._keep = rows, cu, src, sel, keep


def attach_lengths(text: torch.Tensor, lengths) -> torch.Tensor:
    text._ce_lengths = np.ascontiguousarray(np.asarray(lengths, dtype=np.int64).reshape(-1))
    return text


def host_lengths(text_cpu: torch.Tensor) -> np.ndarray:
    return text_cpu.reshape(-1, text_cpu.shape[-1]).numpy().argmax(axis=-1).astype(np.int64) + 1


def tokens_to_device(text: torch.Tensor, device) -> torch.Tensor:
    if text.is_cuda:
        return text
    lens = getattr(text, "_ce_lengths", None)
    if lens is None:
        lens = host_lengths(text)
    if torch.device(device).type == "cuda" and not text.is_pinned():
        pin = torch.empty(text.shape, dtype=text.dtype, pin_memory=True)
        pin.copy_(text)
        text = pin
    out = text.to(device, non_blocking=True)
    out._ce_lengths = lens
    return out


_PACK_CACHE_SLOTS = 8


def _pack_key(text):
    base = text._base if text._base is not None else text
    return (id(base), text.storage_offset(), tuple(text.shape), tuple(text.stride()), text._version), base


def text_packing(model, text, lengths=None) -> TextPacking:
    cl, s = lib(), stream()
    n, T = text.shape
    dev = text.device
    if lengths is None:
        lengths = getattr(text, "_ce_lengths", None)
    cache = getattr(model, "_pack_cache", None)
    if not isinstance(cache, dict):
        cache = model._pack_cache = {}
    key, base = _pack_key(text)
    key = key + (bool(model.pack_text),)
    hit = cache.get(key)
# ... 229 lines not shown
        cl, s = lib(), stream()
        dev = model._flat.device
        if text.device != dev:
            raise RuntimeError("text must live on the model's GPU")
        if text.dtype != torch.int64:
            text = text.long()
        text = text.contiguous()
        n, T = text.shape
        if T != model.context_length:
            raise RuntimeError(f"expected {model.context_length} tokens per row, got {T}")
        D = model.transformer.width
        P = model._pmap
        pk = text_packing(model, text)
        M = pk.rows
        sdt, ST = _stream_type(model)
        x0 = _empty((M, D), sdt, dev)
        check(cl.ce_token_embed_t(ptr(text), ptr(pk.src), ptr(P["token_embedding.weight"]), ptr(P["positional_embedding"]),
                                  ptr(x0), ST, M, T, D, model.vocab_size, s), "ce_token_embed")
        rows = pk.sel
        xN = _empty((n, D), sdt, dev)
        if infer:
            _tower_forward_infer(model, model._tdesc, "text", n, M, pk.cu, x0, xN, rows)
        else:
            lease = _tower_workspace(model, model._tdesc, n, "text")
            check(cl.ce_tower_forward(ctypes.byref(model._tdesc), n, M, ptr(pk.cu), ptr(x0), ptr(lease.buf), ptr(xN), ptr(rows),
                                      s), "ce_tower_forward(text)")
        feat, hfin, mean_f, rstd_f = _tower_top_forward(model, xN, "ln_final", "text_projection")
        if infer:
            return feat
        ctx.model, ctx.lease, ctx.n = model, lease, n
        ctx.stream16 = sdt == torch.float16
        ctx.main_stream = getattr(model, "_main_stream", None)
        ctx.saved = (text, x0, xN, pk, hfin, mean_f, rstd_f)
        return feat

    @staticmethod
    def backward(ctx, dfeat):
        model, lease, n = ctx.model, ctx.lease, ctx.n
        if lease.buf is None:
            raise RuntimeError("backward through encode_text a second time: the activation stash was released")
        cl, s = lib(), stream()
        text, x0, xN, pk, hfin, mean_f, rstd_f = ctx.saved
        dev = model._flat.device
        T, D = model.context_length, model.transformer.width
        M, rows = pk.rows, pk.sel
        model._attach_grads()
        G = model._gview
        _check_stream(ctx, model)
        dxn, gs = _tower_top_backward(model, model._tdesc, _f32(dfeat), xN, hfin, mean_f, rstd_f, "ln_final", "text_projection")
        dx = _empty((M, D), xN.dtype, dev)
        stop = _tower_backward(model, model._tdesc, "text", n, M, pk.cu, x0, lease, dx, rows, dxn)
        lease.release()
        if stop > 0:
            return _tower_backward_done(ctx, "text", 4)
        if gs is not None:
            dx = ops.cast_scaled(dx, torch.float32, gs, divide=True)
        if pk.cu is None:
            check(cl.ce_batch_reduce(ptr(dx), ptr(G("positional_embedding")), n, T * D, T * D, 1, s), "ce_batch_reduce(text pos)")
        else:
            check(cl.ce_pos_embed_bwd_packed(ptr(dx), ptr(pk.cu), ptr(G("positional_embedding")), n, T, D, s),
                  "ce_pos_embed_bwd_packed")
        check(cl.ce_token_embed_bwd(ptr(text), ptr(pk.src), ptr(dx), ptr(G("token_embedding.weight")), M, D, model.vocab_size, s),
              "ce_token_embed_bwd")
        return _tower_backward_done(ctx, "text", 4)


def _sgemm(A, sam, sak, Bm, sbk, sbn, C, M, N, K, alpha_ptr=None, alpha=1.0, alpha_exp=0, beta=0.0):
    check(lib().ce_sgemm(ptr(A), sam, sak, ptr(Bm), sbk, sbn, ptr(C), C.stride(0), M, N, K, ptr(alpha_ptr), alpha, alpha_exp,
                         beta, stream()), "ce_sgemm")


def _l2norm(f):
    n, E = f.shape
    y, inv = torch.empty_like(f), _empty((n,), torch.float32, f.device)
    check(lib().ce_l2norm_fwd(ptr(f), E, ptr(y), E, ptr(inv), n, E, stream()), "ce_l2norm_fwd")
    return y, inv


def _l2norm_bwd(dy, y, inv):
    n, E = y.shape
    df = torch.empty_like(y)
    check(lib().ce_l2norm_bwd(ptr(dy), E, ptr(y), E, ptr(inv), ptr(df), E, n, E, 0, stream()), "ce_l2norm_bwd")
    return df


def _index64(t, dev):
    return None if t is None else t.to(device=dev, dtype=torch.int64).contiguous()


def _infonce_workspace(nq: int, dev):
    return _empty((lib().ce_infonce_workspace_bytes(nq),), torch.uint8, dev)


def _small_head_workspace(nI: int, nT: int, nsel: int, E: int, dev):
    cl = lib()
    return (_empty((cl.ce_head_small_workspace_floats(nI, nT, nsel, E),), torch.float32, dev),
            cl.ce_head_small_scalars_offset(nI, nT, nsel, E))


class LogitsFn(torch.autograd.Function):

    @staticmethod
    def forward(ctx, fi, ft, logit_scale, overbatch: bool, want: str = "both"):
        cl, s = lib(), stream()
        dev = fi.device
        ctx.set_materialize_grads(False)
        fi, ft = _f32(fi), _f32(ft)
        B, E = fi.shape
        N = ft.shape[0]
        In, inv_i = _l2norm(fi)
        Tn, inv_t = _l2norm(ft)
        ls = logit_scale.detach().reshape(1)
        lpt = None
        ctx.twin = want == "both" and overbatch and os.environ.get("CE_HEAD_TWIN", "1") != "0"
        if want in ("both", "text") and not ctx.twin:
            lpt = _empty((N, B), torch.float32, dev)
# ... 329 lines not shown
```

clip_event_amd/model.py:

```python
from __future__ import annotations

import contextlib
import ctypes
import math
import os
from ctypes import c_int, c_void_p
from typing import Dict, List, Optional, Sequence, Tuple

import numpy as np
import torch
from torch import nn

from . import _lib as L
from ._lib import check, lib, ptr, stream
from .utils_image import patch_from_norm_bbox



class _BlockParams(ctypes.Structure):
    _fields_ = [(n, c_void_p) for n in (
        "ln1_w", "ln1_b", "ln2_w", "ln2_b", "b_qkv", "b_out", "b_fc", "b_proj",
        "w_qkv", "w_out", "w_fc", "w_proj", "wt_qkv", "wt_out", "wt_fc", "wt_proj",
        "g_ln1_w", "g_ln1_b", "g_ln2_w", "g_ln2_b", "g_b_qkv", "g_b_out", "g_b_fc", "g_b_proj",
        "g_w_qkv", "g_w_out", "g_w_fc", "g_w_proj",
        "w8_qkv", "w8_out", "w8_fc", "w8_proj", "s8_qkv", "s8_out", "s8_fc", "s8_proj",
        "wt8_qkv", "wt8_out", "wt8_fc", "wt8_proj", "st8_qkv", "st8_out", "st8_fc", "st8_proj")]


class _TowerDesc(ctypes.Structure):
    _fields_ = [("layers", c_int), ("width", c_int), ("heads", c_int), ("tokens", c_int), ("causal", c_int),
                ("blocks", ctypes.POINTER(_BlockParams)), ("fp8", c_int), ("stream16", c_int), ("wgrad_overwrite", c_int), ("grad_scale", c_void_p)]



class _Affine(nn.Module):
    def __init__(self, d: int, bias_init: float = 0.0):
        super().__init__()
        self.weight = nn.Parameter(torch.ones(d))
        self.bias = nn.Parameter(torch.zeros(d))


class _Linear(nn.Module):
    def __init__(self, d_in: int, d_out: int):
        super().__init__()
        bound = 1.0 / math.sqrt(d_in)
        self.weight = nn.Parameter(torch.empty(d_out, d_in).uniform_(-bound, bound))
        self.bias = nn.Parameter(torch.empty(d_out).uniform_(-bound, bound))


class _MHAParams(nn.Module):
    def __init__(self, d: int):
        super().__init__()
        self.in_proj_weight = nn.Parameter(torch.empty(3 * d, d))
        nn.init.xavier_uniform_(self.in_proj_weight)
        self.in_proj_bias = nn.Parameter(torch.zeros(3 * d))
        self.out_proj = _Linear(d, d)
        with torch.no_grad():
            self.out_proj.bias.zero_()


class _MLP(nn.Module):
    def __init__(self, d: int):
        super().__init__()
        self.c_fc = _Linear(d, 4 * d)
        self.c_proj = _Linear(4 * d, d)


class ResidualAttentionBlock(nn.Module):
    def __init__(self, d_model: int, n_head: int):
        super().__init__()
        self.attn = _MHAParams(d_model)
        self.ln_1 = _Affine(d_model)
        self.mlp = _MLP(d_model)
        self.ln_2 = _Affine(d_model)
        self.n_head = n_head


class Transformer(nn.Module):
    def __init__(self, width: int, layers: int, heads: int):
        super().__init__()
        self.width, self.layers, self.heads = width, layers, heads
        self.resblocks = nn.ModuleList([ResidualAttentionBlock(width, heads) for _ in range(layers)])


# ... 72 lines not shown
            "+-65504 clamp; the affected step(s) used a clipped activation / gradient.  Set model.stream16 = False "
            "(CE_STREAM16=0: fp32 streams, as the reference) or, for the gradient stream, lower CE_GRAD_TARGET.")



_GEMM_SUFFIXES = ("attn.in_proj_weight", "attn.out_proj.weight", "mlp.c_fc.weight", "mlp.c_proj.weight")


TOWERS = ("visual", "text")
_INPUT_SIDE = {"visual": ("visual.ln_pre.", "visual.conv1.", "visual.positional_embedding", "visual.class_embedding"),
               "text": ("token_embedding.", "positional_embedding")}
SEGMENT, CHUNK = 2048, 1 << 16


def tower_of(name: str) -> str:
    if name.startswith("visual."):
        return "visual"
    return "text" if name.startswith(("transformer.", "token_embedding.", "positional_embedding", "ln_final.", "text_projection")) else "head"


def block_of(name: str):
    parts = name.split(".")
    return int(parts[parts.index("resblocks") + 1]) if "resblocks" in parts else None


def trainable_tables(offsets, shapes, flags, group_of=None, tile_names=()):
    group_of = group_of or {}
    names = sorted(offsets, key=lambda n: offsets[n])
    numel = {n: int(np.prod(shapes[n], dtype=np.int64)) if len(shapes[n]) else 1 for n in names}
    layers = {t: 1 + max([block_of(n) for n in names if tower_of(n) == t and block_of(n) is not None], default=-1) for t in TOWERS}
    locked, stop = {}, {}
    for t in TOWERS:
        live = [n for n in names if tower_of(n) == t and flags[n]]
        locked[t] = not live
        if any(n.startswith(_INPUT_SIDE[t]) for n in live):
            stop[t] = 0
        else:
            stop[t] = min([block_of(n) for n in live if block_of(n) is not None], default=layers[t])
    tile_set = set(tile_names)
    tiles = [(n, int(group_of.get(n, 0))) for n in tile_names if flags[n]]
    segments, segment_group, chunks = [], [], []
    for n in names:
        if not flags[n]:
            continue
        lo, hi = offsets[n], offsets[n] + (numel[n] + 3) // 4 * 4
        for c in range(lo, hi, CHUNK):
            chunks.append((c, min(c + CHUNK, hi)))
        if n not in tile_set:
            for c in range(lo, hi, SEGMENT):
                segments.append((c, min(c + SEGMENT, hi)))
                segment_group.append(int(group_of.get(n, 0)))
    return {"locked": locked, "stop_layer": stop, "tiles": tiles, "segments": segments, "segment_group": segment_group,
            "chunks": chunks}


class TrainablePlan:

    def __init__(self, flags, tables):
        self.flags = flags
        self.plain = all(flags)
        self.locked, self.stop_layer = tables["locked"], tables["stop_layer"]
        self.host = tables
        self.tjobs = self.segments = self.segment_group = self.chunks = None


class CLIP(nn.Module):

    def __init__(self, embed_dim: int, image_resolution: int, vision_layers: int, vision_width: int,
                 vision_patch_size: int, context_length: int, vocab_size: int, transformer_width: int,
                 transformer_heads: int, transformer_layers: int, constrastive_overbatch=True, alignment=False,
                 multiattention=False):
        super().__init__()
        if isinstance(vision_layers, (tuple, list)):
            raise NotImplementedError("ModifiedResNet towers are out of scope (BASELINE.json names ViT only)")
        self.context_length = context_length
        self.vision_width = vision_width
        self.embed_dim = embed_dim
        vision_heads = vision_width // 64
        self.visual = VisualTransformer(image_resolution, vision_patch_size, vision_width, vision_layers,
                                        vision_heads, embed_dim)
        self.transformer = Transformer(transformer_width, transformer_layers, transformer_heads)
        self.vocab_size = vocab_size
        self.token_embedding = _Embedding(vocab_size, transformer_width)
        self.positional_embedding = nn.Parameter(torch.empty(context_length, transformer_width))
        self.ln_final = _Affine(transformer_width)
        self.text_projection = nn.Parameter(torch.empty(transformer_width, embed_dim))
        self.logit_scale = nn.Parameter(torch.ones([]) * np.log(1 / 0.07))
        self.initialize_parameters()
        self.constrastive_overbatch = constrastive_overbatch
        self.alignment = alignment
        self.multiattention = multiattention
        from .losses import cross_entropy
        self.loss_func = cross_entropy
        self._flat: Optional[torch.Tensor] = None
        self._flat_grad: Optional[torch.Tensor] = None
        self._pool = _Pool()
        self._trigger = None
        self._versions = None
        self.grad_sync = None
        self.pack_text = os.environ.get("CE_TEXT_PACK", "1") != "0"
        self.fp8 = int(os.environ.get("CE_FP8", "0"))
        self.stream16 = os.environ.get("CE_STREAM16", "1") != "0"
        self.grad_target = float(os.environ.get("CE_GRAD_TARGET", "64"))
        self.patch_seed = 0
        self.patch_draw = 0

    _RUNTIME = ("_flat", "_flat_grad", "_flat16", "_offsets", "_ranges", "_layer_end", "_pmap", "_pool", "_trigger",
                "_versions", "_w16", "_w16t", "_kp", "_kp_real", "_conv_pad", "_conv_gpad", "_cast_list", "_tjobs",
                "_tjobs_bwd", "_adam_tiles_ok", "_wt_fresh", "_wt_event", "_aux_stream", "_mirror_fresh", "_mirror_versions", "_vdesc", "_tdesc", "_vblocks", "_tblocks",
                "_side_streams", "_main_stream", "_pack_cache", "_cls_rows", "_sat", "_sat_poll", "_step_events", "grad_sync", "_w8", "_fp8_fresh", "_zero_table", "_zero_tables", "_adam_segs", "_first_touch", "_lease_batch", "_plist", "_plans", "_patch_pin", "_patch_off")

    def __getstate__(self):
        state = dict(self.__dict__)
        for k in self._RUNTIME:
            state.pop(k, None)
        return state

    def __setstate__(self, state):
        super().__setstate__(state)
        self._flat = None
        self._flat_grad = None
        self._pool = _Pool()
        self._trigger = None
        self._versions = None
        self.grad_sync = None
        for p in self.parameters():
            p.grad = None

    def set_hyps(self, constrastive_overbatch=True, alignment=False, multiattention=False):
        self.constrastive_overbatch = constrastive_overbatch
        self.alignment = alignment
        self.multiattention = multiattention

    def enable_logit_bias(self, init: float = -10.0):
        if getattr(self, "logit_bias", None) is not None:
            with torch.no_grad():
                self.logit_bias.fill_(float(init))
            return self.logit_bias
        dev = self.logit_scale.device
        self.logit_bias = nn.Parameter(torch.full([], float(init), dtype=torch.float32, device=dev))
        for k in ("_plist", "_plans"):
            self.__dict__.pop(k, None)
        if self._flat is not None:
            state = self.__getstate__()
            self.__dict__.clear()
            self.__setstate__(state)
        return self.logit_bias

    def load_state_dict(self, state_dict, strict: bool = True, **kw):
        if getattr(self, "logit_bias", None) is not None and "logit_bias" not in state_dict:
            state_dict = dict(state_dict)
            state_dict["logit_bias"] = self.logit_bias.detach().clone()
        return super().load_state_dict(state_dict, strict=strict, **kw)

    def initialize_parameters(self):
        nn.init.normal_(self.token_embedding.weight, std=0.02)
        nn.init.normal_(self.positional_embedding, std=0.01)
        w, layers = self.transformer.width, self.transformer.layers
        proj_std = (w ** -0.5) * ((2 * layers) ** -0.5)
        attn_std = w ** -0.5
        fc_std = (2 * w) ** -0.5
        for block in self.transformer.resblocks:
            nn.init.normal_(block.attn.in_proj_weight, std=attn_std)
# ... 102 lines not shown
                p.grad = self._gview(n)
        else:
            for n, p in todo:
                view = self._gview(n)
                if p.grad is None:
                    view.zero_()
                else:
                    view.copy_(p.grad)
                p.grad = view
        cur = torch.cuda.current_stream()
        for s_ in (getattr(self, "_side_streams", None) or ()):
            if s_ != cur:
                s_.wait_stream(cur)
        ms = getattr(self, "_main_stream", None)
        if ms is not None and ms != cur:
            ms.wait_stream(cur)

    _BLOCK_WEIGHTS = ("attn.in_proj_weight", "attn.out_proj.weight", "mlp.c_fc.weight", "mlp.c_proj.weight")

    def _is_block_weight(self, name: str) -> bool:
        return "resblocks." in name and name.endswith(self._BLOCK_WEIGHTS)

    def _zero_table_for(self):
        if getattr(self, "_zero_tables", None) is None:
            keep = sorted((self._offsets[n], self._offsets[n] + self._pmap[n].numel()) for n in self._pmap if self._is_block_weight(n))
            segs, pos = [], 0
            for lo, hi in keep:
                if lo > pos:
                    segs.append((pos, lo))
                pos = (hi + 63) // 64 * 64
            if pos < self._flat_grad.numel():
                segs.append((pos, self._flat_grad.numel()))
            chunks = []
            for lo, hi in segs:
                for c in range(lo, hi, 1 << 16):
                    chunks.append((c, min(c + (1 << 16), hi)))
            self._zero_tables = torch.tensor(chunks, dtype=torch.int64).reshape(-1, 2).to(self._flat_grad.device)
        return self._zero_tables

    def _adam_segment_table(self):
        if getattr(self, "_adam_segs", None) is None:
            rows = []
            for lo, hi in self._zero_table_for().tolist():
                for c in range(lo, hi, 2048):
                    rows.append((c, min(c + 2048, hi)))
            self._adam_segs = torch.tensor(rows, dtype=torch.int64).reshape(-1, 2).to(self._flat_grad.device)
        return self._adam_segs

    def _zero_segments(self, table):
        if table.shape[0]:
            check(lib().ce_zero_segments(ptr(self._flat_grad), ptr(table), table.shape[0], stream()), "ce_zero_segments")

    def zero_grad_first_touch(self):
        if self._flat_grad is None or os.environ.get("CE_WGRAD_FIRST_TOUCH", "1") == "0":
            return self.zero_grad()
        self._zero_segments(self._zero_table_for())
        self._attach_grads_fast()
        self._first_touch = {"visual", "text"}

    def _settle_first_touch(self):
        pending = getattr(self, "_first_touch", None)
        if not pending:
            return
        for n, p in self._pmap.items():
            if p.requires_grad and self._is_block_weight(n) and (("visual" in pending and n.startswith("visual.")) or
                                                                 ("text" in pending and not n.startswith("visual."))):
                self._gview(n).zero_()
        self._first_touch = set()

    def zero_grad(self, set_to_none: bool = False):
        self._first_touch = set()
        if self._flat_grad is not None and not set_to_none:
            self._flat_grad.zero_()
            self._attach_grads_fast()
        else:
            super().zero_grad(set_to_none=set_to_none)

    def _attach_grads_fast(self):
        base = self._flat_grad.data_ptr()
        for n, p in self._pmap.items():
            if not p.requires_grad:
                if p.grad is not None and p.grad.data_ptr() == base + self._offsets[n] * 4:
                    p.grad = None
            elif p.grad is None or p.grad.data_ptr() != base + self._offsets[n] * 4:
                p.grad = self._gview(n)

    def _flags(self):
        ps = self.__dict__.get("_plist")
        if ps is None:
            ps = self.__dict__["_plist"] = [p for _, p in self.named_parameters()]
        return tuple(p.requires_grad for p in ps)

    def trainable_plan(self, group_of=None, tiles: bool = True) -> TrainablePlan:
        flags = self._flags()
        flat = self._flat if self._flat is not None and self._flat_ok() else None
        key = (flags, tuple(sorted(group_of.items())) if group_of else None, bool(tiles), None if flat is None else flat.data_ptr())
        plans = self.__dict__.setdefault("_plans", {})
        plan = plans.get(key)
        if plan is not None:
            return plan
        named = list(self.named_parameters())
        fl = {n: f for (n, _), f in zip(named, flags)}
        if flat is None:
            offsets, off = {}, 0
            for n, p in named:
                offsets[n] = off
                off += (p.numel() + 63) // 64 * 64
            tile_names = []
        else:
            offsets = self._offsets
            tile_names = [n for n in self._pmap if n.endswith(_GEMM_SUFFIXES)] if tiles else []
        tables = trainable_tables(offsets, {n: tuple(p.shape) for n, p in named}, fl, group_of, tile_names)
        if flat is None:
            tables = {"locked": tables["locked"], "stop_layer": tables["stop_layer"]}
        plan = TrainablePlan(flags, tables)
        if flat is not None:
            dev = flat.device
            plan.tjobs = self._job_table([n for n, _ in tables["tiles"]], [g for _, g in tables["tiles"]])
            plan.segments = torch.tensor(tables["segments"], dtype=torch.int64).reshape(-1, 2).to(dev)
            plan.segment_group = torch.tensor(tables["segment_group"], dtype=torch.int32).to(dev)
            plan.chunks = torch.tensor(tables["chunks"], dtype=torch.int64).reshape(-1, 2).to(dev)
        if len(plans) >= 8:
            plans.clear()
        plans[key] = plan
# ... 432 lines not shown
```

clip_event_amd/optim.py:

```python
from __future__ import annotations

import contextlib
import math
import os
from bisect import bisect_right
import ctypes
from ctypes import c_float, c_int
from typing import List, Sequence

import torch

from ._lib import check, lib, ptr, stream

MAX_GROUPS = 8


class OptimGroup(ctypes.Structure):
    _fields_ = [("lr", c_float), ("weight_decay", c_float), ("decoupled", c_int), ("pad_", c_int)]


def ema_rate(decay: float, warmup: bool, updates: int) -> float:
    d = float(decay)
    if warmup:
        d = min(d, (1.0 + updates) / (10.0 + updates))
    return 1.0 - d


class _FusedFlatOptimizer(torch.optim.Optimizer):

    _GROUP_KEYS = ("lr", "weight_decay")

    def __init__(self, model, max_norm, defaults, groups=None):
        name = type(self).__name__
        named = list(model.named_parameters())
        frozen = [n for n, p in named if not p.requires_grad]
        if (frozen or groups) and not hasattr(model, "trainable_plan"):
            what = f"frozen parameters ({frozen[:3]}...)" if frozen else "parameter groups"
            raise NotImplementedError(f"{name} updates the whole flat parameter buffer; {what} need a model that describes its "
                                      f"trainable ranges (trainable_plan), or {self._stock} over the trainable ones instead")
        if (frozen or groups) and getattr(getattr(model, "grad_sync", None), "plan", None) is not None:
            raise NotImplementedError(f"{name}: the sharded optimiser step (CE_SHARDED_ADAM) does not take frozen parameters or "
                                      "parameter groups")
        self.model = model
        self.max_norm = max_norm
        self.step_count = 0
        self.sat_poll_every = int(os.environ.get("CE_SAT_POLL_EVERY", "16"))
        self.sumsq = None
        self.ema = None
        self.ema_decay, self.ema_warmup, self.ema_updates = None, False, 0
        self._ema_of = None
        self._averaging = False
        by_id, known = {id(p): n for n, p in named}, {n for n, _ in named}
        if len(groups or ()) > MAX_GROUPS:
            raise ValueError(f"{name}: at most {MAX_GROUPS} parameter groups (got {len(groups)})")
        specs, owner = [], {}
        for gi, g in enumerate(groups or ()):
            if not isinstance(g, dict) or "params" not in g:
                raise ValueError(f"{name}: group {gi} must be a dict with a 'params' list")
            extra = sorted(set(g) - {"params"} - set(self._GROUP_KEYS))
            if extra:
                raise ValueError(f"{name}: group {gi} sets {extra}; a group may set {sorted(self._GROUP_KEYS)} only "
                                 "(everything else is shared by all groups)")
            for q in g["params"]:
                n = q if isinstance(q, str) else by_id.get(id(q))
                if n not in known:
                    raise ValueError(f"{name}: group {gi} names {q if isinstance(q, str) else 'a tensor'!r}, which is no parameter of the model")
                if n in owner:
                    raise ValueError(f"{name}: parameter {n} is in groups {owner[n]} and {gi}")
                if n in frozen:
                    raise ValueError(f"{name}: group {gi} names the frozen parameter {n}; unfreeze it first")
                owner[n] = gi
            specs.append((self._group_hyper(g), {n for n, at in owner.items() if at == gi}))
        if not specs or any(p.requires_grad and n not in owner for n, p in named):
            specs.insert(0, ({}, None))
        if len(specs) > MAX_GROUPS:
            raise ValueError(f"{name}: at most {MAX_GROUPS} parameter groups (got {len(specs)} with the unnamed parameters' group)")
        self._specs = specs
        self._flags_seen = tuple(p.requires_grad for _, p in named)
        if groups or frozen:
            params = [{"params": [p for n, p in named if p.requires_grad and (n in names if names is not None else n not in owner)],
                       **hyper} for hyper, names in specs]
        else:
            params = [p for _, p in named]
        super().__init__(params, defaults)

    def _group_hyper(self, g):
        return {k: g[k] for k in ("lr", "weight_decay") if k in g}

    def _follow_flags(self):
        m = self.model
        if not hasattr(m, "_flags"):
            return
        flags = m._flags()
        if flags == self._flags_seen:
            return
        named = list(m.named_parameters())
        owner = {n: gi for gi, (_, names) in enumerate(self._specs) for n in names or ()}
        woken = [n for (n, p), was in zip(named, self._flags_seen) if p.requires_grad and not was]
        if all(names is not None for _, names in self._specs) and any(p.requires_grad and n not in owner for n, p in named):
            if len(self._specs) >= MAX_GROUPS:
                raise ValueError(f"{type(self).__name__}: a parameter unfrozen outside every group needs the unnamed parameters' "
                                 f"group, and there are {MAX_GROUPS} groups already")
            self._specs.append(({}, None))
            self.add_param_group({"params": [p for n, p in named if p.requires_grad and n not in owner]})
        for g, (_, names) in zip(self.param_groups, self._specs):
            g["params"] = [p for n, p in named if p.requires_grad and (n in names if names is not None else n not in owner)]
        self._flags_seen = flags
        if woken and self.step_count > 0 and getattr(m, "_flat", None) is not None:
            for buf in self.state_buffers():
                for n in woken:
                    o = m._offsets[n]
                    buf[o:o + (m._pmap[n].numel() + 63) // 64 * 64].zero_()

    def _group_of(self):
        owner = {n: gi for gi, (_, names) in enumerate(self._specs) for n in names or ()}
        default = next((gi for gi, (_, names) in enumerate(self._specs) if names is None), None)
        return {n: owner.get(n, default) for n, p in self.model.named_parameters() if p.requires_grad}

    def _plain(self) -> bool:
        return len(self.param_groups) == 1 and not self.param_groups[0].get("decoupled_weight_decay") and all(self._flags_seen)

    def _grouped_step(self, sumsq, s):
        m = self.model
        if getattr(getattr(m, "grad_sync", None), "plan", None) is not None:
            raise NotImplementedError(f"{type(self).__name__}: the sharded optimiser step (CE_SHARDED_ADAM) does not take frozen "
                                      "parameters or parameter groups")
        group_of = self._group_of()
        if not group_of:
            raise RuntimeError(f"{type(self).__name__}.step: every parameter is frozen")
        tiles = bool(getattr(m, "_adam_tiles_ok", False)) and os.environ.get("CE_ADAM_TILES", "1") != "0"
        plan = m.trainable_plan(group_of, tiles=tiles)
        garr = (OptimGroup * len(self.param_groups))()
        for i, g in enumerate(self.param_groups):
            garr[i].lr, garr[i].weight_decay, garr[i].decoupled = float(g["lr"]), float(g["weight_decay"]), int(bool(g.get("decoupled_weight_decay")))
        if sumsq is not None:
            sumsq.zero_()
            check(lib().ce_sumsq_segments(ptr(m._flat_grad), ptr(plan.chunks), plan.chunks.shape[0], ptr(sumsq), s),
                  "ce_sumsq_segments")
        state, args = self._group_args(sumsq)
        tj, tn_, tt = plan.tjobs
        suffix, ema = self._ema_args()
        check(getattr(lib(), self._groups_op + suffix)(ptr(m._flat), ptr(m._flat_grad), *(ptr(b) for b in state), ptr(m._flat16),
                                                       ptr(tj), tn_, tt, ptr(plan.segments), plan.segments.shape[0],
                                                       ptr(plan.segment_group), ptr(sumsq), self.max_norm or 0.0, garr,
                                                       len(garr), *args, *ema, s), self._groups_op + suffix)
        m.mark_operands_stale(mirror_fresh=True, wt_fresh=tiles)

    @property
    def ema_enabled(self) -> bool:
        return self.ema_decay is not None

    def _refuse_while_averaged(self, what):
        if self._averaging:
            raise RuntimeError(f"{type(self).__name__}.{what} inside averaged(): the model holds the averaged weights; leave the "
                               "context first")

    def enable_ema(self, decay: float = 0.9999, warmup: bool = False):
        self._refuse_while_averaged("enable_ema")
        decay = float(decay)
        if not 0.0 <= decay < 1.0:
            raise ValueError(f"{type(self).__name__}.enable_ema: decay must lie in [0, 1) (got {decay})")
        self.ema_decay, self.ema_warmup = decay, bool(warmup)
        self.ema = self._ema_of = None
        self._state()
        self._ema_ready()

    def disable_ema(self):
        self._refuse_while_averaged("disable_ema")
        self.ema = self._ema_of = None
        self.ema_decay, self.ema_warmup, self.ema_updates = None, False, 0

    def _ema_ready(self):
        flat = self.model._flat
        if self.ema_enabled and (self.ema is None or self._ema_of is not flat):
            self.ema = flat.detach().clone()
            self._ema_of = flat
            self.ema_updates = 0

    def _ema_args(self, lo=None, hi=None):
        if not self.ema_enabled:
            return "", ()
        e = self.ema if lo is None else self.ema[lo:hi]
        return "_ema", (ptr(e), ema_rate(self.ema_decay, self.ema_warmup, self.ema_updates))

    def _swap_average(self):
        m = self.model
        m.wait_transposes()
        check(lib().ce_swap_cast_bf16(ptr(m._flat), ptr(self.ema), ptr(m._flat16), m._flat.numel(), stream()), "ce_swap_cast_bf16")
# ... 7 lines not shown
        self._state()
        self._ema_ready()
        self._swap_average()
        self._averaging = True
        try:
            yield self.model
        finally:
            self._averaging = False
            self._swap_average()

    def _named_offsets(self):
        m = self.model
        return [(n, p, m._offsets[n]) for n, p in m.named_parameters()]

    def ema_state_dict(self):
        if not self.ema_enabled:
            raise RuntimeError(f"{type(self).__name__}.ema_state_dict: EMA is off")
        if not self._averaging:
            self._state()
            self._ema_ready()
        src = self.model._flat if self._averaging else self.ema
        shadow = {n: src[o:o + p.numel()].view(p.shape).clone() for n, p, o in self._named_offsets()}
        return {"decay": self.ema_decay, "warmup": self.ema_warmup, "updates": self.ema_updates, "shadow": shadow}

    def load_ema_state_dict(self, sd):
        self._refuse_while_averaged("load_ema_state_dict")
        shadow = sd["shadow"]
        named = {n: p for n, p in self.model.named_parameters()}
        missing, extra = sorted(set(named) - set(shadow)), sorted(set(shadow) - set(named))
        if missing or extra:
            raise ValueError(f"EMA state does not match the model: missing {missing[:3]}, unexpected {extra[:3]}")
        for n, p in named.items():
            if tuple(shadow[n].shape) != tuple(p.shape):
                raise ValueError(f"EMA state does not match the model: {n} is {tuple(shadow[n].shape)}, expected {tuple(p.shape)}")
        self.enable_ema(sd["decay"], sd.get("warmup", False))
        with torch.no_grad():
            for n, p, o in self._named_offsets():
                self.ema[o:o + p.numel()].view(p.shape).copy_(shadow[n])
        self.ema_updates = int(sd.get("updates", 0))

    @property
    def lr(self):
        return self.param_groups[0]["lr"]

    @property
    def weight_decay(self):
        return self.param_groups[0]["weight_decay"]

    def zero_grad(self, set_to_none: bool = False):
        self._state()
        self.model._flat_grad.zero_()
        self.model._attach_grads_fast()

    def zero_grad_first_touch(self):
        self._state()
        self.model.zero_grad_first_touch()

    def grad_norm(self) -> torch.Tensor:
        return self.sumsq.sqrt()

    @torch.no_grad()
    def step(self, closure=None):
        if closure is not None:
            raise RuntimeError(f"{type(self).__name__}.step takes no closure")
        self._refuse_while_averaged("step")
        self._state()
        self._ema_ready()
        m = self.model
        self._follow_flags()
        m._settle_first_touch()
        m.wait_transposes()
        n = m._flat.numel()
        s = stream()
        self.step_count += 1
        from . import distributed as D
        plan = getattr(getattr(m, "grad_sync", None), "plan", None)
        sharded = plan is not None and D.active()
        if sharded and self.ema_enabled:
            raise NotImplementedError(f"{type(self).__name__}: the sharded optimiser step (CE_SHARDED_ADAM) does not carry the weight "
                                      "EMA; use the replicated step (every rank then computes the same average)")
        sumsq = self.sumsq if self.max_norm is not None else None
        if not self._plain():
            self._grouped_step(sumsq, s)
            self._after_step(False)
            self.ema_updates += int(self.ema_enabled)
            if self.sat_poll_every and self.step_count % self.sat_poll_every == 0 and hasattr(m, "poll_stream16_saturation"):
                m.poll_stream16_saturation()
            return
        state, args = self._step_args(sumsq)

        def sum_squares(lo, hi):
            check(lib().ce_sumsq(ptr(m._flat_grad[lo:hi]), hi - lo, ptr(self.sumsq), s), "ce_sumsq")

        def update(lo, hi):
            suffix, ema = self._ema_args(lo, hi)
            check(getattr(lib(), self._flat_op + suffix)(ptr(m._flat[lo:hi]), ptr(m._flat_grad[lo:hi]),
                                                         *(ptr(b if b is None else b[lo:hi]) for b in state),
                                                         ptr(m._flat16[lo:hi]), hi - lo, *args, *ema, s), self._flat_op + suffix)

        if sharded:
            D.sharded_update(plan, m._flat, sumsq, sum_squares, update)
            m.mark_operands_stale(mirror_fresh=False)
        else:
            if sumsq is not None:
                sumsq.zero_()
                sum_squares(0, n)
            if getattr(m, "_adam_tiles_ok", False) and os.environ.get("CE_ADAM_TILES", "1") != "0":
                tj, tn_, tt = m._tjobs_bwd
                seg = m._adam_segment_table()
                suffix, ema = self._ema_args()
                check(getattr(lib(), self._tiles_op + suffix)(ptr(m._flat), ptr(m._flat_grad), *(ptr(b) for b in state), ptr(m._flat16),
                                                              ptr(tj), tn_, tt, ptr(seg), seg.shape[0], *args, *ema, s),
                      self._tiles_op + suffix)
                m.mark_operands_stale(mirror_fresh=True, wt_fresh=True)
            else:
                update(0, n)
                m.mark_operands_stale(mirror_fresh=True)
        self._after_step(sharded)
        self.ema_updates += int(self.ema_enabled)
        if self.sat_poll_every and self.step_count % self.sat_poll_every == 0 and hasattr(m, "poll_stream16_saturation"):
            m.poll_stream16_saturation()

    def _params(self):
        self._follow_flags()
        return [p for g in self.param_groups for p in g["params"]]

    def _offset_of(self):
        names = {id(p): n for n, p in self.model.named_parameters()}
        return [self.model._offsets[names[id(p)]] for p in self._params()]

    def _pieces(self, buf):
        return [buf[o:o + p.numel()].view(p.shape) for p, o in zip(self._params(), self._offset_of())]

    def _state_dict_of(self, state):
        self._params()
        groups, at = [], 0
        for g in self.param_groups:
            group = {k: v for k, v in g.items() if k != "params"}
            group["params"] = list(range(at, at + len(g["params"])))
            at += len(g["params"])
            groups.append(group)
        return {"state": state, "param_groups": groups}

    def _refuse_sharded_state(self, what):
        if getattr(self, "_moments_stale", False):
            raise RuntimeError(f"the {what} sharded over the ranks (sharded optimiser step): call "
                               "clip_event_amd.distributed.consolidate(model, optimizer) on EVERY rank before state_dict()")

    def _matching_group(self, sd):
        self._params()
        groups = sd["param_groups"]
        if len(self.param_groups) == 1:
            params = self.param_groups[0]["params"]
            if len(groups) != 1 or len(groups[0]["params"]) != len(params):
                raise ValueError("optimizer state does not match: expected one group of %d parameters" % len(params))
            return groups[0]
        if len(groups) != len(self.param_groups) or any(len(a["params"]) != len(b["params"]) for a, b in zip(groups, self.param_groups)):
# ... 341 lines not shown
```

include/clip_event_hip.h:

```cpp
#ifndef CLIP_EVENT_HIP_H
#define CLIP_EVENT_HIP_H

#include <stddef.h>
#include <stdint.h>

#ifdef __cplusplus
extern "C" {
#endif

const char* ce_last_error(void);
int ce_version(void);

enum {
    CE_EPI_BF16 = 0,
    CE_EPI_F32 = 1,
    CE_EPI_BIAS_BF16 = 2,
    CE_EPI_BIAS_F32 = 3,
    CE_EPI_BIAS_RESID_F32 = 4,
    CE_EPI_BIAS_GELU = 5,
    CE_EPI_GELUGRAD_BF16 = 6,
    CE_EPI_BIAS_RESID_F16 = 7,
    CE_EPI_BIAS_QGELU_BF16 = 8
};

#ifndef CE_T_F32
#define CE_T_F32 0
#define CE_T_BF16 1
#define CE_T_F16 2
#endif

int ce_gemm_nt(const void* A, long lda, const void* B, long ldb, int M, int N, int K, int epilogue,
               const float* bias, const void* resid, long ldr, void* out, long ldo, void* out2, long ldo2,
               const void* aux, long ldaux, void* stream);

int ce_gemm_tn(const void* P, long ldp, const void* Q, long ldq, int M, int Nn, int Kk, float* out, long ldo,
               int splits, void* stream);
int ce_gemm_tn_bias(const void* P, long ldp, const void* Q, long ldq, int M, int Nn, int Kk, float* out, long ldo,
                    float* bias_grad, int splits, void* stream);
#define CE_TN_MAX_GROUP 36
int ce_gemm_tn_grouped(int count, const void* const* P, const long* ldp, const void* const* Q, const long* ldq, int M,
                       const int* Nn, const int* Kk, float* const* out, const long* ldo, int splits, void* stream);
int ce_gemm_tn_grouped_ex(int count, const void* const* P, const long* ldp, const void* const* Q, const long* ldq, int M,
                          const int* Nn, const int* Kk, float* const* out, const long* ldo, int splits, int overwrite,
                          void* stream);

int ce_quant_rows_fp8(const void* x, long ldx, void* q, long ldq, float* scale, int M, int K, void* stream);
typedef struct ce_quant_job {
    const void* src; void* dst; float* scale;
    long lds_; long ldd;
    int rows, cols;
    int group_start, pad_;
} ce_quant_job;
int ce_quant_rows_fp8_multi(const ce_quant_job* jobs_device, int njobs, int total_groups, void* stream);
int ce_gemm_nt_fp8(const void* A8, long lda, const float* sa, const void* B8, long ldb, const float* sb, int M, int N,
                   int K, int epilogue, const float* bias, const void* resid, long ldr, void* out, long ldo, void* out2,
                   long ldo2, const void* aux, long ldaux, void* stream);
int ce_quant_mx_fp8(const void* x, long ldx, void* q, long ldq, void* scale8, long lds_, int M, int K, void* stream);
int ce_quant_mx_fp8_multi(const ce_quant_job* jobs_device, int njobs, int total_groups, void* stream);
int ce_gemm_nt_mx8(const void* A8, long lda, const void* sa8, const void* B8, long ldb, const void* sb8, int M, int N, int K,
                   int epilogue, const float* bias, const void* resid, long ldr, void* out, long ldo, void* out2, long ldo2,
                   const void* aux, long ldaux, void* stream);
int ce_layernorm_fwd(const float* x, long ldx, const int* rows, const float* w, const float* b, void* y, long ldy,
                     int out_f32, float* mean, float* rstd, int M, int D, float eps, void* stream);
int ce_layernorm_fwd_t(const void* x, int x_type, long ldx, const int* rows, const float* w, const float* b, void* y,
                       int y_type, long ldy, float* mean, float* rstd, int M, int D, float eps, void* stream);

int ce_layernorm_fwd_q8(const void* x, int x_type, long ldx, const int* rows, const float* w, const float* b, void* y,
                        int y_type, long ldy, float* mean, float* rstd, int M, int D, float eps, void* q8, long ldq,
                        float* qscale, void* stream);

int ce_layernorm_bwd(const void* dy, long lddy, int dy_f32, const float* x, long ldx, const int* rows,
                     const float* mean, const float* rstd, const float* w, const float* dx_in, float* dx_out,
                     long lddx, void* dxb, long lddxb, float* dw, float* db, float* dxsum, int M, int D,
                     void* stream);
int ce_layernorm_bwd_t(const void* dy, int dy_type, long lddy, const void* x, int x_type, long ldx, const int* rows,
                       const float* mean, const float* rstd, const float* w, const void* dx_in, int dxin_type,
                       void* dx_out, int dx_type, long lddx, void* dxb, long lddxb, float* dw, float* db, float* dxsum,
                       const float* gscale, int M, int D, void* stream);

int ce_layernorm_bwd_q8(const void* dy, int dy_type, long lddy, const void* x, int x_type, long ldx, const int* rows,
                        const float* mean, const float* rstd, const float* w, const void* dx_in, int dxin_type,
                        void* dx_out, int dx_type, long lddx, void* dxb, long lddxb, float* dw, float* db, float* dxsum,
                        const float* gscale, int M, int D, void* q8, long ldq, float* qscale, void* stream);

int ce_layernorm_bwd_blocks(int M, int D);
int ce_layernorm_bwd_partials(const void* dy, int dy_type, long lddy, const void* x, int x_type, long ldx, const int* rows,
                              const float* mean, const float* rstd, const float* w, const void* dx_in, int dxin_type,
                              void* dx_out, int dx_type, long lddx, void* dxb, long lddxb, int want_dxsum,
                              const float* gscale, int M, int D, void* q8, long ldq, float* qscale, float* partials,
                              void* stream);
#define CE_LN_FOLD_MAX 64
typedef struct ce_ln_fold_job {
    const float* partials;
    float *dw, *db, *dxsum;
    int blocks, D;
} ce_ln_fold_job;
int ce_layernorm_fold(const ce_ln_fold_job* jobs , int njobs, void* stream);
// ... 38 lines not shown
                         int M, int row_bytes, void* stream);
int ce_eot_rows(const int64_t* ids, int* rows, long n, int tokens, void* stream);

typedef struct {
    const unsigned char* src;
    long pitch;
    int x0, y0, w, h;
    int ow, oh;
    int left, top;
    int row0, rows;
    long tmp_off;
} ce_preproc_desc;
size_t ce_preprocess_table_bytes(int n_out, int n_px, int kmax);
int ce_preprocess(const ce_preproc_desc* descs_device, int n_out, int n_px, int kmax, int max_rows, void* table,
                  void* tmp, float* out, const float* mean, const float* std, void* stream);

enum { CE_AUG_BRIGHTNESS = 0, CE_AUG_CONTRAST = 1, CE_AUG_SATURATION = 2, CE_AUG_HUE = 3 };
typedef struct {
    int flip;
    int grey;
    int n_ops;
    int op[4];
    float factor[4];
} ce_augment_desc;
size_t ce_augment_workspace_bytes(int n_out, int n_px, int kmax, long tmp_bytes);
int ce_augment(const ce_preproc_desc* descs_device, const ce_augment_desc* augs_device, const ce_augment_desc* augs_host,
               int n_out, int n_px, int kmax, int max_rows, void* workspace, float* out, const float* mean, const float* std,
               void* stream);

int ce_l2norm_fwd(const float* f, long ldf, float* y, long ldy, float* inv_norm, int n, int E, void* stream);
int ce_l2norm_bwd(const float* dy, long lddy, const float* y, long ldy, const float* inv_norm, float* df, long lddf,
                  int n, int E, int accumulate, void* stream);
int ce_sgemm(const float* A, long sam, long sak, const float* B, long sbk, long sbn, float* C, long ldc, int M,
             int N, int K, const float* alpha_ptr, float alpha, int alpha_exp, float beta, void* stream);
int ce_xent_fwd(const float* logits, long ld, const int64_t* labels, const int64_t* sel, float* row_lse,
                float* loss, int nrows, int C, void* stream);
int ce_xent_bwd(const float* logits, long ld, const int64_t* labels, const int64_t* sel, const float* row_lse,
                const float* grad, float* dlogits, long ldd, int nrows, int C, void* stream);
int ce_soft_xent_fwd(const float* logits, long ld, const float* teacher_logits, long ldt, const int64_t* sel, float* row_lse,
                     float* row_lse_t, float* loss, int nrows, int C, void* stream);
int ce_soft_xent_bwd(const float* logits, long ld, const float* teacher_logits, long ldt, const int64_t* sel,
                     const float* row_lse, const float* row_lse_t, const float* grad, float* dlogits, long ldd, int nrows,
                     int C, void* stream);
int ce_dot(const float* a, const float* b, long n, float* out, void* stream);
int ce_instance_logits(const float* In, const float* Tn, const float* logit_scale, float* lpi, int B, int K, int E,
                       void* stream);
int ce_instance_logits_bwd(const float* dlpi, const float* In, const float* Tn, const float* logit_scale, float* dIn,
                           float* dTn, int B, int K, int E, void* stream);
int ce_elem_loss_fwd(const float* x, const float* y, long n, int mode, float* loss, void* stream);
int ce_elem_loss_bwd(const float* x, const float* y, long n, int mode, const float* grad, float* dx, void* stream);

int ce_sumsq(const float* g, long n, float* out, void* stream);
int ce_zero_segments(float* base, const long* table_device, int nchunks, void* stream);
int ce_adam_step(float* p, const float* g, float* m, float* v, void* p_bf16, long n, const float* sumsq, float max_norm,
                 float lr, float beta1, float beta2, float eps, float weight_decay, int step, void* stream);
typedef struct ce_transpose_job {
    const void* src;
    void* dst;
    int rows, cols, tile_start, pad_;
} ce_transpose_job;
int ce_multi_transpose_bf16(const ce_transpose_job* jobs_device, int njobs, int total_tiles, void* stream);
int ce_adam_step_tiles(float* p, const float* g, float* m, float* v, void* p_bf16, const ce_transpose_job* jobs_device, int njobs,
                       int total_tiles, const long* segments_device, int nsegments, const float* sumsq, float max_norm, float lr,
                       float beta1, float beta2, float eps, float weight_decay, int step, void* stream);
int ce_sgd_step(float* p, const float* g, float* buf, void* p_bf16, long n, const float* sumsq, float max_norm, float lr,
                float momentum, float dampening, float weight_decay, int nesterov, int first_step, void* stream);
int ce_sgd_step_tiles(float* p, const float* g, float* buf, void* p_bf16, const ce_transpose_job* jobs_device, int njobs,
                      int total_tiles, const long* segments_device, int nsegments, const float* sumsq, float max_norm, float lr,
                      float momentum, float dampening, float weight_decay, int nesterov, int first_step, void* stream);
int ce_sumsq_segments(const float* g, const long* table_device, int nchunks, float* out, void* stream);
typedef struct ce_optim_group {
    float lr, weight_decay;
    int decoupled, pad_;
} ce_optim_group;
int ce_adam_step_groups(float* p, const float* g, float* m, float* v, void* p_bf16, const ce_transpose_job* jobs_device, int njobs,
                        int total_tiles, const long* segments_device, int nsegments, const int* segment_group, const float* sumsq,
                        float max_norm, const ce_optim_group* groups, int ngroups, float beta1, float beta2, float eps, int step,
                        void* stream);
int ce_sgd_step_groups(float* p, const float* g, float* buf, void* p_bf16, const ce_transpose_job* jobs_device, int njobs,
                       int total_tiles, const long* segments_device, int nsegments, const int* segment_group, const float* sumsq,
                       float max_norm, const ce_optim_group* groups, int ngroups, float momentum, float dampening, int nesterov,
                       int first_step, void* stream);
int ce_adam_step_ema(float* p, const float* g, float* m, float* v, void* p_bf16, long n, const float* sumsq, float max_norm,
                     float lr, float beta1, float beta2, float eps, float weight_decay, int step, float* ema, float ema_rate,
                     void* stream);
int ce_adam_step_tiles_ema(float* p, const float* g, float* m, float* v, void* p_bf16, const ce_transpose_job* jobs_device, int njobs,
                           int total_tiles, const long* segments_device, int nsegments, const float* sumsq, float max_norm, float lr,
                           float beta1, float beta2, float eps, float weight_decay, int step, float* ema, float ema_rate,
                           void* stream);
int ce_adam_step_groups_ema(float* p, const float* g, float* m, float* v, void* p_bf16, const ce_transpose_job* jobs_device, int njobs,
                            int total_tiles, const long* segments_device, int nsegments, const int* segment_group, const float* sumsq,
                            float max_norm, const ce_optim_group* groups, int ngroups, float beta1, float beta2, float eps, int step,
                            float* ema, float ema_rate, void* stream);
int ce_sgd_step_ema(float* p, const float* g, float* buf, void* p_bf16, long n, const float* sumsq, float max_norm, float lr,
                    float momentum, float dampening, float weight_decay, int nesterov, int first_step, float* ema, float ema_rate,
                    void* stream);
int ce_sgd_step_tiles_ema(float* p, const float* g, float* buf, void* p_bf16, const ce_transpose_job* jobs_device, int njobs,
                          int total_tiles, const long* segments_device, int nsegments, const float* sumsq, float max_norm, float lr,
                          float momentum, float dampening, float weight_decay, int nesterov, int first_step, float* ema,
                          float ema_rate, void* stream);
int ce_sgd_step_groups_ema(float* p, const float* g, float* buf, void* p_bf16, const ce_transpose_job* jobs_device, int njobs,
                           int total_tiles, const long* segments_device, int nsegments, const int* segment_group, const float* sumsq,
                           float max_norm, const ce_optim_group* groups, int ngroups, float momentum, float dampening, int nesterov,
                           int first_step, float* ema, float ema_rate, void* stream);
int ce_lion_step(float* p, const float* g, float* m, void* p_bf16, long n, const float* sumsq, float max_norm, float lr,
                 float beta1, float beta2, float weight_decay, void* stream);
int ce_lion_step_tiles(float* p, const float* g, float* m, void* p_bf16, const ce_transpose_job* jobs_device, int njobs,
                       int total_tiles, const long* segments_device, int nsegments, const float* sumsq, float max_norm, float lr,
                       float beta1, float beta2, float weight_decay, void* stream);
int ce_lion_step_groups(float* p, const float* g, float* m, void* p_bf16, const ce_transpose_job* jobs_device, int njobs,
                        int total_tiles, const long* segments_device, int nsegments, const int* segment_group, const float* sumsq,
                        float max_norm, const ce_optim_group* groups, int ngroups, float beta1, float beta2, void* stream);
int ce_lion_step_ema(float* p, const float* g, float* m, void* p_bf16, long n, const float* sumsq, float max_norm, float lr,
                     float beta1, float beta2, float weight_decay, float* ema, float ema_rate, void* stream);
int ce_lion_step_tiles_ema(float* p, const float* g, float* m, void* p_bf16, const ce_transpose_job* jobs_device, int njobs,
                           int total_tiles, const long* segments_device, int nsegments, const float* sumsq, float max_norm, float lr,
                           float beta1, float beta2, float weight_decay, float* ema, float ema_rate, void* stream);
int ce_lion_step_groups_ema(float* p, const float* g, float* m, void* p_bf16, const ce_transpose_job* jobs_device, int njobs,
                            int total_tiles, const long* segments_device, int nsegments, const int* segment_group, const float* sumsq,
                            float max_norm, const ce_optim_group* groups, int ngroups, float beta1, float beta2, float* ema,
                            float ema_rate, void* stream);
int ce_swap_cast_bf16(float* a, float* b, void* a_bf16, long n, void* stream);

typedef struct ce_block_params {
    const float *ln1_w, *ln1_b, *ln2_w, *ln2_b;
    const float *b_qkv, *b_out, *b_fc, *b_proj;
    const void *w_qkv, *w_out, *w_fc, *w_proj;
    const void *wt_qkv, *wt_out, *wt_fc, *wt_proj;
    float *g_ln1_w, *g_ln1_b, *g_ln2_w, *g_ln2_b;
    float *g_b_qkv, *g_b_out, *g_b_fc, *g_b_proj;
    float *g_w_qkv, *g_w_out, *g_w_fc, *g_w_proj;
    const void *w8_qkv, *w8_out, *w8_fc, *w8_proj;
    const float *s8_qkv, *s8_out, *s8_fc, *s8_proj;
    const void *wt8_qkv, *wt8_out, *wt8_fc, *wt8_proj;
    const float *st8_qkv, *st8_out, *st8_fc, *st8_proj;
} ce_block_params;

typedef struct ce_tower_desc {
    int layers, width, heads, tokens, causal;
    const ce_block_params* blocks;
    int fp8;
    int stream16;
    int wgrad_overwrite;
    const float* grad_scale;
} ce_tower_desc;

size_t ce_tower_workspace_bytes(const ce_tower_desc* d, int batch);
int ce_tower_forward(const ce_tower_desc* d, int batch, int rows, const int* cu_seqlens, const void* x0,
                     void* workspace, void* x_out, const int* sel_rows, void* stream);
size_t ce_tower_infer_workspace_bytes(const ce_tower_desc* d, int batch);
int ce_tower_forward_infer(const ce_tower_desc* d, int batch, int rows, const int* cu_seqlens, const void* x0,
                           void* workspace, void* x_out, const int* sel_rows, void* stream);
int ce_tower_backward(const ce_tower_desc* d, int batch, int rows, const int* cu_seqlens, const void* x0,
                      void* workspace, void* dx, const int* sel_rows, const float* dx_sel, void* stream);
int ce_tower_backward_range(const ce_tower_desc* d, int batch, int rows, const int* cu_seqlens, const void* x0,
                            void* workspace, void* dx, const int* sel_rows, const float* dx_sel, int layer_hi,
                            int layer_lo, void* stream);

int ce_ot_fwd(const float* txt, long tsb, long tsr, const float* img, long isb, long isr,
              const unsigned char* txt_pad, const unsigned char* img_pad, float* dist, float* T, float* txt_inv,
              float* img_inv, int B, int M, int N, int D, float beta, int iters, void* stream);
int ce_ot_bwd(const float* txt, long tsb, long tsr, const float* img, long isb, long isr, const float* T,
              const float* txt_inv, const float* img_inv, const float* grad, float* dtxt, float* dimg, int B, int M,
              int N, int D, void* stream);
int ce_bbox_pool_fwd(const float* grid, long sb, long s0, long s1, const int* boxes, float* out, int nbox, int E,
                     void* stream);
int ce_bbox_pool_bwd(const float* dout, const int* boxes, float* dgrid, int g, int nbox, int E, void* stream);

#define CE_INFONCE_MAX_SPLITS 64
size_t ce_infonce_workspace_bytes(int nq);
int ce_infonce_fwd(const float* q, long ldq, const int64_t* sel, int nq, const float* k, long ldk, int nk, int E,
                   const float* logit_scale, const int64_t* labels, float* lse, float* loss, void* workspace, void* stream);
int ce_infonce_bwd(const float* q, long ldq, const int64_t* sel, int nq, const float* k, long ldk, int nk, int E,
                   const float* logit_scale, const int64_t* labels, const float* lse, const float* grad, float* dq, float* dk,
                   float* dlogit_scale, void* stream);

size_t ce_sigmoid_head_workspace_bytes(int nq, int nk);
int ce_sigmoid_head_fwd(const float* q, long ldq, const int64_t* sel, int nq, const float* k, long ldk, int nk, int E,
                        const float* logit_scale, const float* logit_bias, const int64_t* labels, float* loss, void* workspace,
                        void* stream);
int ce_sigmoid_head_bwd(const float* q, long ldq, const int64_t* sel, int nq, const float* k, long ldk, int nk, int E,
                        const float* logit_scale, const float* logit_bias, const int64_t* labels, const float* grad, float* dq,
                        float* dk, float* dlogit_scale, float* dlogit_bias, void* stream);

size_t ce_distill_head_workspace_bytes(int nq);
int ce_distill_head_fwd(const float* q, long ldq, const int64_t* sel, int nq, const float* k, long ldk, int nk, int Es,
                        const float* logit_scale, const float* tq, long ldtq, const float* tk, long ldtk, int Et,
                        const float* teacher_logit_scale, float* lse_s, float* lse_t, float* v, float* loss, void* workspace,
                        void* stream);
int ce_distill_head_bwd(const float* q, long ldq, const int64_t* sel, int nq, const float* k, long ldk, int nk, int Es,
                        const float* logit_scale, const float* tq, long ldtq, const float* tk, long ldtk, int Et,
                        const float* teacher_logit_scale, const float* lse_s, const float* lse_t, const float* v,
                        const float* grad, float* dq, float* dk, void* stream);
int ce_rowdot_sum(const float* x, long ldx, const float* y, long ldy, int n, int E, float* out, void* stream);

#define CE_TOPK_MAX 16
size_t ce_score_topk_workspace_bytes(int nq, int nk, int k, int splits);
int ce_score_topk(const float* q, long ldq, int nq, const float* keys, long ldk, int nk, int E, const float* logit_scale,
                  const int64_t* target, int k, int splits, float* top_val, int64_t* top_idx, float* lse, int64_t* rank,
                  void* workspace, void* stream);

size_t ce_head_small_workspace_floats(int nI, int nT, int nsel, int E);
size_t ce_head_small_scalars_offset(int nI, int nT, int nsel, int E);
int ce_head_small_fwd(const float* fi, const float* ft, int nI, int nT, int E, const float* logit_scale, const int64_t* labels_i,
                      const int64_t* labels_t, const int64_t* sel, int nsel, float* workspace, void* stream);
int ce_head_small_bwd(int nI, int nT, int nsel, int E, const float* logit_scale, const float* g_i, const float* g_t,
                      const int64_t* sel, const float* workspace, float* dfi, float* dft, float* dlogit_scale, void* stream);

int ce_region_nce_fwd(const float* region, const float* desc, const float* label, const int* offsets, int groups,
                      int max_rows, int E, const float* logit_scale, int use_label, int role_text, float* loss_bbox,
                      float* loss_arg, void* stream);
int ce_region_nce_bwd(const float* region, const float* desc, const float* label, const int* offsets, int groups,
                      int max_rows, int E, const float* logit_scale, int use_label, int role_text, const float* g_bbox,
                      const float* g_arg, float* dregion, float* ddesc, float* dlabel, float* dlogit_scale, void* stream);

#define CE_PROF_NT_FAMILIES 8
enum {
    CE_PROF_GEMM_NT0 = 0,
    CE_PROF_GEMM_TN = 64, CE_PROF_ATTN_FWD = 65, CE_PROF_ATTN_BWD = 66, CE_PROF_LN_FWD = 67, CE_PROF_LN_BWD = 68,
    CE_PROF_COLSUM = 69, CE_PROF_OTHER = 70, CE_PROF_GEMM_TN2 = 71 ,
    CE_PROF_GEMM_NT_QGELU = 72,
    CE_PROF_NCLASS = 80
};
void ce_profile_enable(int on);
int ce_profile_collect(double* out, int max_classes);
int ce_profile_num_classes(void);
const char* ce_profile_class_name(int cls);

void ce_gemm_nt_tune(int variant);
int ce_gemm_nt_last_plan(int* tall_panels, int* short_tm);
typedef struct { int kernel, tm, ts, tall_panels, tiles_m, tiles_n, tile_chunk,
                 workgroups, block, lds_bytes, wants_tile_queue, taken; } ce_nt_plan;
int ce_gemm_nt_plan(int M, int N, int K, int epilogue, int fp8,
                    long lda, long ldb, long ldo, long ldo2, long ldaux, long ldr,
                    ce_nt_plan* out);
typedef struct { int variant, force_splits, depth, rows, loader_waves; } ce_tn_knobs;
typedef struct { int form, rows, stages, block, lds_bytes, workgroups, splits, m_per_split, depth,
                 kernel_overwrites, zero_fill_first, tiles, prof_class;
                 int tiles_n[CE_TN_MAX_GROUP], tiles_k[CE_TN_MAX_GROUP], tile_end[CE_TN_MAX_GROUP]; } ce_tn_plan;
int ce_gemm_tn_plan(int count, const int* Nn, const int* Kk, int M, int splits, int overwrite,
                    const ce_tn_knobs* knobs, ce_tn_plan* out);
int ce_tower_wgrad_cuts(int n_blocks, int width, int M, long extra_tiles, int force_group, int* sizes_out);
void ce_gemm_nt_fp8_tune(int variant);

int ce_gemm_set_cu_budget(int cus);
int ce_gemm_set_dynamic_tiles(int on);

int ce_cu_hog(int blocks, float microseconds, void* stream);
double ce_cu_hog_clock_mhz(void);

int ce_probe_mfma(int shape, const void* a_frags, const void* b_frags, float* out, void* stream);
int ce_probe_mfma_scale(const void* a_frags, const void* b_frags, const int* scale_a, const int* scale_b, float* out, void* stream);
int ce_probe_tr16(const void* image, int n_elems, const int* byte_off, void* out, void* stream);

#ifdef __cplusplus
}
#endif
#endif
```

Measured before the change: 21210 pairs/s (whole job).

## Fold gradient-norm sum of squares into weight-gradient GEMM epilogues

The TN weight-gradient GEMM kernels now optionally accumulate the squared sum of their output tiles into a global scalar when the plan overwrites the output with no split-K, so clip_grad_norm only has to run a sumsq pass over the parameter segments that were not folded. The zero-segments kernel also clears the accumulator, and the Python side tracks which segments were folded. It also stops folding LayerNorm partials through the ring every 8 layers, keeping one set per layer and doing a single fold launch. This removes a full re-read of most of the flat gradient buffer, at the cost of a wave reduction plus atomic per wave in the GEMM epilogues and some planning and bookkeeping overhead.

```diff
diff --git a/clip_event_amd/csrc/gemm.hip b/clip_event_amd/csrc/gemm.hip
--- a/clip_event_amd/csrc/gemm.hip
+++ b/clip_event_amd/csrc/gemm.hip
@@ -1300,9 +1300,15 @@
 struct TNGroup {
     int count, splits, m_per_split, M, depth;
     int overwrite = 0;
+    float* sumsq = nullptr;
     int tile_end[CE_TN_MAX_GROUP];
     TNArgs prob[CE_TN_MAX_GROUP];
 };
+
+__device__ __forceinline__ void tn_fold_sumsq(float* acc, float s) {
+    s = wave_sum_dpp(s);
+    if ((threadIdx.x & 63) == 0) atomicAdd(acc, s);
+}
 
 __global__ __launch_bounds__(256, 2) void gemm_tn2_kernel(TNGroup grp) {
     extern __shared__ __attribute__((aligned(16))) char smem[];
@@ -1426,6 +1432,19 @@
                     }
                 }
             }
+        if (grp.sumsq) {
+            float sq[2][2] = {{0.f, 0.f}, {0.f, 0.f}};
+#pragma unroll
+            for (int nt = 0; nt < 2; ++nt)
+#pragma unroll
+                for (int kt = 0; kt < 2; ++kt)
+#pragma unroll
+                    for (int r = 0; r < 16; ++r) {
+                        const int n = en + nt * 32 + (r & 3) + 8 * (r >> 2);
+                        if (n < p.Nn && ek + kt * 32 < p.Kk) sq[nt][kt] = __builtin_fmaf(acc[nt][kt][r], acc[nt][kt][r], sq[nt][kt]);
+                    }
+            tn_fold_sumsq(grp.sumsq, (sq[0][0] + sq[0][1]) + (sq[1][0] + sq[1][1]));
+        }
     }
 }
 
@@ -1556,6 +1575,16 @@
                 else atomicAdd(p.out + (long)n * p.ldo + k, acc[nt][kt][r]);
             }
         }
+    if (grp.sumsq) {
+        float sq[2][2] = {{0.f, 0.f}, {0.f, 0.f}};
+#pragma unroll
+        for (int nt = 0; nt < 2; ++nt)
+#pragma unroll
+            for (int kt = 0; kt < 2; ++kt)
+#pragma unroll
+                for (int r = 0; r < 16; ++r) sq[nt][kt] = __builtin_fmaf(acc[nt][kt][r], acc[nt][kt][r], sq[nt][kt]);
+        tn_fold_sumsq(grp.sumsq, (sq[0][0] + sq[0][1]) + (sq[1][0] + sq[1][1]));
+    }
 }
 
 template <int T3_ROWS, int T3_STAGES>
@@ -1683,6 +1712,17 @@
 
     const int ek = k0 + wk * 64 + (lane & 31);
     const int en = n0 + wn * 128 + 4 * (lane >> 5);
+    if (grp.sumsq) {
+        float sq[4] = {0.f, 0.f, 0.f, 0.f};
+#pragma unroll
+        for (int nt = 0; nt < 4; ++nt)
+#pragma unroll
+            for (int kt = 0; kt < 2; ++kt)
+#pragma unroll
+                for (int r = 0; r < 16; ++r) sq[nt] = __builtin_fmaf(acc[nt][kt][r], acc[nt][kt][r], sq[nt]);
+        tn_fold_sumsq(grp.sumsq, (sq[0] + sq[1]) + (sq[2] + sq[3]));
+    }
+    __builtin_amdgcn_sched_barrier(0);
 #pragma unroll
     for (int nt = 0; nt < 4; ++nt)
 #pragma unroll
@@ -1964,6 +2004,12 @@
 extern "C" int ce_gemm_tn_grouped_ex(int count, const void* const* P, const long* ldp, const void* const* Q,
                                      const long* ldq, int M, const int* Nn, const int* Kk, float* const* out,
                                      const long* ldo, int splits, int overwrite, void* stream) {
+    return ce_gemm_tn_grouped_acc(count, P, ldp, Q, ldq, M, Nn, Kk, out, ldo, splits, overwrite, nullptr, stream);
+}
+
+extern "C" int ce_gemm_tn_grouped_acc(int count, const void* const* P, const long* ldp, const void* const* Q,
+                                      const long* ldq, int M, const int* Nn, const int* Kk, float* const* out,
+                                      const long* ldo, int splits, int overwrite, float* sumsq_acc, void* stream) {
     CE_CHECK_ARG(count >= 1 && count <= CE_TN_MAX_GROUP && M > 0, "ce_gemm_tn_grouped: 1..%d problems, M > 0", CE_TN_MAX_GROUP);
     hipStream_t s = (hipStream_t)stream;
     TNGroup g;
@@ -1988,6 +2034,7 @@
 
     const TNPlan p = tn_plan(M, count, Nn, Kk, splits, overwrite != 0, tn_process_knobs());
     g.splits = p.splits; g.m_per_split = p.m_per_split; g.depth = p.depth; g.overwrite = p.kernel_overwrites;
+    g.sumsq = tn_plan_folds(p) ? sumsq_acc : nullptr;
     for (int i = 0; i < CE_TN_MAX_GROUP; ++i) g.tile_end[i] = p.tile_end[i];
     for (int i = 0; i < count; ++i) {
         TNArgs& a = g.prob[i];
@@ -2035,6 +2082,16 @@
     return 0;
 }
 
+extern "C" int ce_gemm_tn_folds(int count, const int* Nn, const int* Kk, int M, int splits, int overwrite, const ce_tn_knobs* knobs,
+                                int* folded_out) {
+    CE_CHECK_ARG(folded_out && Nn && Kk && count >= 1 && count <= CE_TN_MAX_GROUP && M > 0,
+                 "ce_gemm_tn_folds: 1..%d problems, M > 0 and a result array", CE_TN_MAX_GROUP);
+    for (int i = 0; i < count; ++i) CE_CHECK_ARG(Nn[i] > 0 && Kk[i] > 0, "ce_gemm_tn_folds: empty problem %d", i);
+    const bool f = tn_plan_folds(tn_plan(M, count, Nn, Kk, splits, overwrite != 0, knobs ? TNKnobs(*knobs) : tn_process_knobs()));
+    for (int i = 0; i < count; ++i) folded_out[i] = f ? 1 : 0;
+    return 0;
+}
+
 extern "C" int ce_probe_mfma(int shape, const void* a_frags, const void* b_frags, float* out, void* stream) {
     if (shape == 16)
         hipLaunchKernelGGL(probe_mfma16_kernel, dim3(1), dim3(64), 0, (hipStream_t)stream, (const bf16x8*)a_frags,
diff --git a/clip_event_amd/csrc/optim.hip b/clip_event_amd/csrc/optim.hip
--- a/clip_event_amd/csrc/optim.hip
+++ b/clip_event_amd/csrc/optim.hip
@@ -337,7 +337,9 @@
     }
 }
 
-__global__ __launch_bounds__(256) void zero_segments_kernel(float* __restrict__ base, const long* __restrict__ table) {
+__global__ __launch_bounds__(256) void zero_segments_kernel(float* __restrict__ base, const long* __restrict__ table,
+                                                            float* __restrict__ scalar) {
+    if (scalar && blockIdx.x == 0 && threadIdx.x == 0) *scalar = 0.f;
     const long lo = table[2 * blockIdx.x], hi = table[2 * blockIdx.x + 1];
     for (long i = lo + threadIdx.x * 4; i < hi; i += 1024)
         __builtin_nontemporal_store(f32x4{0.f, 0.f, 0.f, 0.f}, reinterpret_cast<f32x4*>(base + i));
@@ -586,8 +588,12 @@
 }
 
 extern "C" int ce_zero_segments(float* base, const long* table_device, int nchunks, void* stream) {
+    return ce_zero_segments_scalar(base, table_device, nchunks, nullptr, stream);
+}
+
+extern "C" int ce_zero_segments_scalar(float* base, const long* table_device, int nchunks, float* scalar, void* stream) {
     CE_CHECK_ARG(base && table_device && nchunks > 0, "ce_zero_segments: empty");
-    hipLaunchKernelGGL(zero_segments_kernel, dim3(nchunks), dim3(256), 0, (hipStream_t)stream, base, table_device);
+    hipLaunchKernelGGL(zero_segments_kernel, dim3(nchunks), dim3(256), 0, (hipStream_t)stream, base, table_device, scalar);
     CE_LAUNCH_CHECK();
     return 0;
 }
@@ -596,6 +602,7 @@
     CE_CHECK_ARG(n > 0, "ce_sumsq: empty");
     long blocks = (n + 1023) / 1024;
     if (blocks > 2048) blocks = 2048;
+    CeProfScope prof(CE_PROF_GRAD_NORM, 0.0, 4.0 * n, (hipStream_t)stream);
     hipLaunchKernelGGL(sumsq_kernel, dim3((unsigned)blocks), dim3(256), 0, (hipStream_t)stream, g, n, out);
     CE_LAUNCH_CHECK();
     return 0;
@@ -805,6 +812,7 @@
 
 extern "C" int ce_sumsq_segments(const float* g, const long* table_device, int nchunks, float* out, void* stream) {
     CE_CHECK_ARG(g && table_device && out && nchunks > 0, "ce_sumsq_segments: empty");
+    CeProfScope prof(CE_PROF_GRAD_NORM, 0.0, 0.0, (hipStream_t)stream);
     hipLaunchKernelGGL(sumsq_segments_kernel, dim3((unsigned)nchunks), dim3(256), 0, (hipStream_t)stream, g, table_device, out);
     CE_LAUNCH_CHECK();
     return 0;
diff --git a/clip_event_amd/csrc/tn_plan.cpp b/clip_event_amd/csrc/tn_plan.cpp
--- a/clip_event_amd/csrc/tn_plan.cpp
+++ b/clip_event_amd/csrc/tn_plan.cpp
@@ -105,3 +105,39 @@
     for (int k = n; k > 0; k -= take[k]) sizes_out[groups++] = take[k];
     return groups;
 }
+
+void tn_tower_folds(int layers, int width, int M, int batch, bool pruned, int layer_hi, int layer_lo, bool overwrite,
+                    int force_group, const TNKnobs& knobs, unsigned char* folded) {
+    const int w = width, last = layers - 1;
+    for (int i = 0; i < 4 * layers; ++i) folded[i] = 0;
+    int id[CE_TN_MAX_GROUP], Nn[CE_TN_MAX_GROUP], Kk[CE_TN_MAX_GROUP], count = 0;
+    auto queue = [&](int which, int n, int k) { id[count] = which; Nn[count] = n; Kk[count] = k; ++count; };
+    auto flush = [&](int rows) {
+        if (count == 0) return;
+        if (tn_plan_folds(tn_plan(rows, count, Nn, Kk, 0, overwrite, knobs)))
+            for (int i = 0; i < count; ++i) folded[id[i]] = 1;
+        count = 0;
+    };
+    int top = layer_hi;
+    if (layer_hi == last && pruned) {
+        queue(4 * last + 0, w, 4 * w); queue(4 * last + 1, 4 * w, w); queue(4 * last + 2, w, w);
+        flush(batch);
+        queue(4 * last + 3, 3 * w, w);
+        top = last - 1;
+    }
+    bool cut_after[TN_CUT_MAX_BLOCKS] = {};
+    if (top >= layer_lo) {
+        int sizes[TN_CUT_MAX_BLOCKS];
+        const int groups = tn_group_cuts(top - layer_lo + 1, w, M, count > 0 ? 3 * tn_problem_tiles(M, w, w) : 0, force_group, sizes);
+        int l = top;
+        for (int i = 0; i < groups; ++i) {
+            l -= sizes[i];
+            cut_after[l + 1] = true;
+        }
+    }
+    for (int l = top; l >= layer_lo; --l) {
+        queue(4 * l + 0, w, 4 * w); queue(4 * l + 1, 4 * w, w); queue(4 * l + 2, w, w); queue(4 * l + 3, 3 * w, w);
+        if (cut_after[l] || count + 4 > CE_TN_MAX_GROUP) flush(M);
+    }
+    flush(M);
+}
diff --git a/clip_event_amd/csrc/tn_plan.hpp b/clip_event_amd/csrc/tn_plan.hpp
--- a/clip_event_amd/csrc/tn_plan.hpp
+++ b/clip_event_amd/csrc/tn_plan.hpp
@@ -33,7 +33,14 @@
 
 TNPlan tn_plan(int M, int count, const int* Nn, const int* Kk, int splits_arg, bool overwrite, const TNKnobs& knobs);
 
+constexpr bool tn_plan_folds(const TNPlan& p) {
+    return (p.kernel_overwrites || p.zero_fill_first) && p.splits == 1 && p.form != TN_V1;
+}
+
 constexpr int TN_CUT_MAX_BLOCKS = 64;
 constexpr int TN_GROUP_MAX_BLOCKS = 8;
 
 int tn_group_cuts(int n_blocks, int width, int M, long extra_tiles, int force_group, int* sizes_out);
+
+void tn_tower_folds(int layers, int width, int M, int batch, bool pruned, int layer_hi, int layer_lo, bool overwrite,
+                    int force_group, const TNKnobs& knobs, unsigned char* folded);
diff --git a/clip_event_amd/csrc/tower.cpp b/clip_event_amd/csrc/tower.cpp
--- a/clip_event_amd/csrc/tower.cpp
+++ b/clip_event_amd/csrc/tower.cpp
@@ -13,6 +13,12 @@
 constexpr int WG_MAX_BLOCKS = TN_GROUP_MAX_BLOCKS;
 constexpr int WG_SETS = WG_MAX_BLOCKS + 1;
 constexpr int LNP_RING = 8;
+constexpr int LNP_ALL_LAYERS = 16;
+int lnp_sets(int layers) {
+    static const int once = getenv("CE_LN_FOLD_ONCE") ? atoi(getenv("CE_LN_FOLD_ONCE")) : 1;
+    if (once && layers <= LNP_ALL_LAYERS) return layers;
+    return layers < LNP_RING ? layers : LNP_RING;
+}
 
 struct Carver {
     char* base;
@@ -43,7 +49,8 @@
     float* q8s;
     float *xs_in, *xs_mid, *dxs_mid, *means, *rstds;
     bf16_t *os, *h2s, *as, *gs, *dxbs, *dxb2s, *das, *dhs, *dos;
-    float* lnp[LNP_RING][2];
+    float* lnp[LNP_ALL_LAYERS][2];
+    int lnp_n;
     size_t bytes;
 };
 
@@ -84,9 +91,10 @@
     L.dxbs = c.take<bf16_t>(Bn * w); L.dxb2s = c.take<bf16_t>(Bn * w); L.das = c.take<bf16_t>(Bn * 4 * w);
     L.dhs = c.take<bf16_t>(Bn * w); L.dos = c.take<bf16_t>(Bn * w);
     const size_t lnp_floats = (size_t)ce_layernorm_bwd_blocks((int)M, (int)w) * 3 * w;
-    for (int l = 0; l < LNP_RING; ++l) {
-        L.lnp[l][0] = l < d->layers ? c.take<float>(lnp_floats) : nullptr;
-        L.lnp[l][1] = l < d->layers ? c.take<float>(lnp_floats) : nullptr;
+    L.lnp_n = lnp_sets(d->layers);
+    for (int l = 0; l < LNP_ALL_LAYERS; ++l) {
+        L.lnp[l][0] = l < L.lnp_n ? c.take<float>(lnp_floats) : nullptr;
+        L.lnp[l][1] = l < L.lnp_n ? c.take<float>(lnp_floats) : nullptr;
     }
     L.bytes = (c.off + 255) & ~size_t(255);
 }
@@ -262,7 +270,8 @@
     const long esz = d->stream16 ? 2 : 4;
     const int last = d->layers - 1;
     static const int ln_fold = getenv("CE_LN_FOLD") ? atoi(getenv("CE_LN_FOLD")) : 1;
-    ce_ln_fold_job fold_jobs[2 * LNP_RING];
+    static_assert(LNP_RING <= LNP_ALL_LAYERS && 2 * LNP_ALL_LAYERS <= CE_LN_FOLD_MAX, "one ce_layernorm_fold launch takes every set");
+    ce_ln_fold_job fold_jobs[2 * LNP_ALL_LAYERS];
     int n_fold = 0;
     int fold_rc = 0;
     const int ln_blocks = ce_layernorm_bwd_blocks(M, w);
@@ -274,7 +283,7 @@
         fold_jobs[n_fold++] = ce_ln_fold_job{partial, dgw, dgb, dxs, ln_blocks, w};
         const int rc = ce_layernorm_bwd_partials(dy, CE_T_BF16, w, xin, ST, w, nullptr, mean, rstd, gamma, dx, ST, dx, ST, w, dxb, w, dxs ? 1 : 0, GS, M, w, q8, w,
                                                  L.q8s, partial, stream);
-        if (rc == 0 && n_fold == 2 * LNP_RING) {
+        if (rc == 0 && n_fold == 2 * L.lnp_n && L.lnp_n < d->layers) {
             fold_rc = ce_layernorm_fold(fold_jobs, n_fold, stream);
             n_fold = 0;
             return fold_rc;
@@ -293,22 +302,37 @@
             cut_after[l + 1] = true;
         }
     };
+    float* const gnorm = d->wgrad_overwrite ? d->gnorm_acc : nullptr;
+    unsigned char folds[4 * Layout::MAX_LAYERS];
+    if (gnorm) tn_tower_folds(d->layers, w, M, batch, sel_rows != nullptr, layer_hi, layer_lo, true, force_group, tn_process_knobs(), folds);
+    auto check_folds = [&](int rows_, int count, const int* Nn, const int* Kk, const int* id) -> int {
+        if (!gnorm) return 0;
+        const bool f = tn_plan_folds(tn_plan(rows_, count, Nn, Kk, 0, true, tn_process_knobs()));
+        for (int i = 0; i < count; ++i)
+            CE_CHECK_ARG((folds[id[i]] != 0) == f, "ce_tower_backward: the fold report disagrees with the launch of weight gradient %d of block %d",
+                         id[i] % 4, id[i] / 4);
+        return 0;
+    };
     struct Pending {
+        int id[CE_TN_MAX_GROUP];
         const void* P[CE_TN_MAX_GROUP]; long ldp[CE_TN_MAX_GROUP];
         const void* Q[CE_TN_MAX_GROUP]; long ldq[CE_TN_MAX_GROUP];
         int Nn[CE_TN_MAX_GROUP], Kk[CE_TN_MAX_GROUP];
         float* out[CE_TN_MAX_GROUP]; long ldo[CE_TN_MAX_GROUP];
         int count = 0, blocks = 0;
     } pend;
-    auto queue = [&](const void* P, long ldp, const void* Q, long ldq, int Nn, int Kk, float* out, long ldo) {
+    auto queue = [&](int id, const void* P, long ldp, const void* Q, long ldq, int Nn, int Kk, float* out, long ldo) {
         const int i = pend.count++;
+        pend.id[i] = id;
         pend.P[i] = P; pend.ldp[i] = ldp; pend.Q[i] = Q; pend.ldq[i] = ldq;
         pend.Nn[i] = Nn; pend.Kk[i] = Kk; pend.out[i] = out; pend.ldo[i] = ldo;
     };
     auto flush = [&]() -> int {
         if (pend.count == 0) return 0;
-        const int rc = ce_gemm_tn_grouped_ex(pend.count, pend.P, pend.ldp, pend.Q, pend.ldq, M, pend.Nn, pend.Kk, pend.out,
-                                             pend.ldo, 0, d->wgrad_overwrite, stream);
+        int rc = check_folds(M, pend.count, pend.Nn, pend.Kk, pend.id);
+        if (rc == 0)
+            rc = ce_gemm_tn_grouped_acc(pend.count, pend.P, pend.ldp, pend.Q, pend.ldq, M, pend.Nn, pend.Kk, pend.out, pend.ldo, 0,
+                                        d->wgrad_overwrite, gnorm, stream);
         pend.count = 0;
         pend.blocks = 0;
         return rc;
@@ -344,9 +368,11 @@
             const int Kk[3] = {4 * w, w, w};
             float* out[3] = {p.g_w_proj, p.g_w_fc, p.g_w_out};
             const long ldo[3] = {4L * w, w, w};
-            TRY(ce_gemm_tn_grouped_ex(3, P, ldp, Q, ldq, Bn, Nn, Kk, out, ldo, 0, d->wgrad_overwrite, stream));
+            const int id[3] = {4 * l + 0, 4 * l + 1, 4 * l + 2};
+            TRY(check_folds(Bn, 3, Nn, Kk, id));
+            TRY(ce_gemm_tn_grouped_acc(3, P, ldp, Q, ldq, Bn, Nn, Kk, out, ldo, 0, d->wgrad_overwrite, gnorm, stream));
         }
-        queue(L.dqkv[q], 3L * w, s.h1, w, 3 * w, w, p.g_w_qkv, w);
+        queue(4 * l + 3, L.dqkv[q], 3L * w, s.h1, w, 3 * w, w, p.g_w_qkv, w);
         TRY(linear(b8, L, q8_of, L.dqkv[q], 3 * w, p.wt_qkv, p.wt8_qkv, p.st8_qkv, M, w, 3 * w, CE_EPI_BF16, nullptr, nullptr, 0, L.dh, w, nullptr, 0,
                        nullptr, 0, stream));
         TRY(ce_scatter_rows_zero(L.dxs_mid, w * esz, dx, w * esz, sel_rows, Bn, M, (int)(w * esz), stream));
@@ -370,26 +396,37 @@
         if (l == last) TRY(ce_colsum_bf16(dxb_a, w, p.g_b_proj, M, w, stream));
         TRY(linear(b8, L, q8_of, da, 4 * w, p.wt_fc, p.wt8_fc, p.st8_fc, M, w, 4 * w, CE_EPI_BF16, nullptr, nullptr, 0, L.dh, w, nullptr, 0,
                        nullptr, 0, stream));
-        TRY(ln_bwd(L.dh, s.x_mid, s.mean2, s.rstd2, p.ln2_w, dxb_b, p.g_ln2_w, p.g_ln2_b, p.g_b_out, lnq ? L.q8 : nullptr, L.lnp[l % LNP_RING][1]));
+        TRY(ln_bwd(L.dh, s.x_mid, s.mean2, s.rstd2, p.ln2_w, dxb_b, p.g_ln2_w, p.g_ln2_b, p.g_b_out, lnq ? L.q8 : nullptr, L.lnp[l % L.lnp_n][1]));
         if (lnq) q8_of = dxb_b;
         TRY(linear(b8, L, q8_of, dxb_b, w, p.wt_out, p.wt8_out, p.st8_out, M, w, w, CE_EPI_BF16, nullptr, nullptr, 0, L.d_o, w, nullptr, 0, nullptr, 0,
                        stream));
         TRY(ce_attention_bwd(s.qkv, 3 * w, s.o, w, L.d_o, w, s.lse, dqkv, 3 * w, p.g_b_qkv, cu_seqlens, batch, d->tokens, d->heads,
                              d->causal, stream));
-        queue(dxb_a, w, s.g, 4L * w, w, 4 * w, p.g_w_proj, 4L * w);
-        queue(da, 4L * w, s.h2, w, 4 * w, w, p.g_w_fc, w);
-        queue(dxb_b, w, s.o, w, w, w, p.g_w_out, w);
-        queue(dqkv, 3L * w, s.h1, w, 3 * w, w, p.g_w_qkv, w);
+        queue(4 * l + 0, dxb_a, w, s.g, 4L * w, w, 4 * w, p.g_w_proj, 4L * w);
+        queue(4 * l + 1, da, 4L * w, s.h2, w, 4 * w, w, p.g_w_fc, w);
+        queue(4 * l + 2, dxb_b, w, s.o, w, w, w, p.g_w_out, w);
+        queue(4 * l + 3, dqkv, 3L * w, s.h1, w, 3 * w, w, p.g_w_qkv, w);
         ++pend.blocks;
         if (cut_after[l] || pend.count + 4 > CE_TN_MAX_GROUP) TRY(flush());
         TRY(linear(b8, L, q8_of, dqkv, 3 * w, p.wt_qkv, p.wt8_qkv, p.st8_qkv, M, w, 3 * w, CE_EPI_BF16, nullptr, nullptr, 0, L.dh, w, nullptr, 0,
                        nullptr, 0, stream));
         TRY(ln_bwd(L.dh, x_in, s.mean1, s.rstd1, p.ln1_w, L.dxb[(l + WG_SETS - 1) % WG_SETS], p.g_ln1_w, p.g_ln1_b,
-                   (l > 0) ? d->blocks[l - 1].g_b_proj : nullptr, (lnq && l > layer_lo) ? L.q8 : nullptr, L.lnp[l % LNP_RING][0]));
+                   (l > 0) ? d->blocks[l - 1].g_b_proj : nullptr, (lnq && l > layer_lo) ? L.q8 : nullptr, L.lnp[l % L.lnp_n][0]));
         if (lnq && l > layer_lo) q8_of = L.dxb[(l + WG_SETS - 1) % WG_SETS];
     }
     TRY(flush());
     if (n_fold > 0) TRY(ce_layernorm_fold(fold_jobs, n_fold, stream));
+    return 0;
+}
+
+extern "C" int ce_tower_backward_folds(const ce_tower_desc* d, int batch, int rows, int pruned, int layer_hi, int layer_lo,
+                                       unsigned char* folded_out) {
+    TRY(check_desc(d, batch));
+    CE_CHECK_ARG(folded_out && rows > 0 && layer_lo >= 0 && layer_lo <= layer_hi && layer_hi < d->layers,
+                 "ce_tower_backward_folds: rows > 0, layers %d..%d inside 0..%d and a result array of 4 * layers", layer_hi, layer_lo, d->layers - 1);
+    static const int force_group = getenv("CE_WGRAD_GROUP") ? atoi(getenv("CE_WGRAD_GROUP")) : 0;
+    tn_tower_folds(d->layers, d->width, rows, batch, pruned != 0, layer_hi, layer_lo, d->wgrad_overwrite != 0, force_group,
+                   tn_process_knobs(), folded_out);
     return 0;
 }
 
diff --git a/clip_event_amd/engine.py b/clip_event_amd/engine.py
--- a/clip_event_amd/engine.py
+++ b/clip_event_amd/engine.py
@@ -377,7 +377,7 @@
     elif teacher_image is not None or teacher_features is not None:
         raise ValueError("teacher_image / teacher_features need distill=Distillation(...)")
     if hasattr(optimizer, "zero_grad_first_touch"):
-        optimizer.zero_grad_first_touch()
+        optimizer.zero_grad_first_touch(fold_norm=not chunked and grad_sync is None and not D.active())
     else:
         optimizer.zero_grad()
     want_align = model.alignment and criterion_ot is not None
diff --git a/clip_event_amd/functional.py b/clip_event_amd/functional.py
--- a/clip_event_amd/functional.py
+++ b/clip_event_amd/functional.py
@@ -65,14 +65,48 @@
     desc.wgrad_overwrite = 1 if (pending and tower in pending) else 0
     if desc.wgrad_overwrite:
         pending.discard(tower)
+    ranges = list(cuts) + [stop] if stop < layers else []
+    _arm_gnorm_fold(model, desc, tower, batch, rows, sel is not None, ranges)
     hi = layers - 1
-    for lo in (list(cuts) + [stop] if stop < layers else []):
+    for lo in ranges:
         check(cl.ce_tower_backward_range(ctypes.byref(desc), batch, rows, ptr(cu), ptr(x0), ptr(lease.buf), ptr(dx), ptr(sel),
                                          ptr(dx_sel), hi, lo, s), f"ce_tower_backward_range({tower})")
         if lo > stop:
             model.grad_sync(model, tower, upto_layer=lo)
         hi = lo - 1
     return stop
+
+
+def _arm_gnorm_fold(model, desc, tower: str, batch: int, rows: int, pruned: bool, ranges):
+    from .model import folded_names
+    desc.gnorm_acc = None
+    gn = getattr(model, "_gnorm", None)
+    if gn is None:
+        return
+    gn["passes"][tower] = gn["passes"].get(tower, 0) + 1
+    if gn["passes"][tower] > 1:
+        gn["dirty"] = True
+        return
+    if not desc.wgrad_overwrite or len(ranges) != 1:
+        return
+    folded = (ctypes.c_ubyte * (4 * desc.layers))()
+    check(lib().ce_tower_backward_folds(ctypes.byref(desc), batch, rows, int(pruned), desc.layers - 1, ranges[0], folded),
+          f"ce_tower_backward_folds({tower})")
+    names = folded_names(tower, folded)
+    if names and all(model._pmap[n].requires_grad for n in names):
+        desc.gnorm_acc = gn["acc"].data_ptr()
+        gn["folded"] |= names
+
+
+def _gnorm_text_piece(model):
+    gn = getattr(model, "_gnorm", None)
+    if gn is None or gn["dirty"] or gn["text_done"] or gn["passes"].get("text") != 1:
+        return
+    table = model._gnorm_chunks("text", gn["folded"], True)
+    if table.shape[0]:
+        check(lib().ce_sumsq_segments(ptr(model._flat_grad), ptr(table), table.shape[0], ptr(gn["acc"]), stream()),
+              "ce_sumsq_segments(text side)")
+    gn["text_done"] = True
 
 
 class TextPacking:
@@ -408,6 +442,7 @@
         stop = _tower_backward(model, model._tdesc, "text", n, M, pk.cu, x0, lease, dx, rows, dxn)
         lease.release()
         if stop > 0:
+            _gnorm_text_piece(model)
             return _tower_backward_done(ctx, "text", 4)
         if gs is not None:
             dx = ops.cast_scaled(dx, torch.float32, gs, divide=True)
@@ -418,6 +453,7 @@
                   "ce_pos_embed_bwd_packed")
         check(cl.ce_token_embed_bwd(ptr(text), ptr(pk.src), ptr(dx), ptr(G("token_embedding.weight")), M, D, model.vocab_size, s),
               "ce_token_embed_bwd")
+        _gnorm_text_piece(model)
         return _tower_backward_done(ctx, "text", 4)
 
 
diff --git a/clip_event_amd/model.py b/clip_event_amd/model.py
--- a/clip_event_amd/model.py
+++ b/clip_event_amd/model.py
@@ -29,7 +29,8 @@
 
 class _TowerDesc(ctypes.Structure):
     _fields_ = [("layers", c_int), ("width", c_int), ("heads", c_int), ("tokens", c_int), ("causal", c_int),
-                ("blocks", ctypes.POINTER(_BlockParams)), ("fp8", c_int), ("stream16", c_int), ("wgrad_overwrite", c_int), ("grad_scale", c_void_p)]
+                ("blocks", ctypes.POINTER(_BlockParams)), ("fp8", c_int), ("stream16", c_int), ("wgrad_overwrite", c_int), ("grad_scale", c_void_p),
+                ("gnorm_acc", c_void_p)]
 
 
 
@@ -208,6 +209,34 @@
                 segment_group.append(int(group_of.get(n, 0)))
     return {"locked": locked, "stop_layer": stop, "tiles": tiles, "segments": segments, "segment_group": segment_group,
             "chunks": chunks}
+
+
+FOLD_SUFFIXES = ("mlp.c_proj.weight", "mlp.c_fc.weight", "attn.out_proj.weight", "attn.in_proj_weight")
+
+
+def folded_names(tower: str, folded) -> set:
+    prefix = "visual.transformer." if tower == "visual" else "transformer."
+    return {f"{prefix}resblocks.{i // 4}.{FOLD_SUFFIXES[i % 4]}" for i, f in enumerate(folded) if f}
+
+
+def gnorm_tables(offsets, shapes, flags, folded=(), text_done: bool = False):
+    folded = set(folded)
+    frozen = sorted(n for n in folded if not flags[n])
+    if frozen:
+        raise ValueError(f"gnorm_tables: folded tensors {frozen[:3]} are frozen")
+    out = {"text": [], "main": []}
+    for n in sorted(offsets, key=lambda n: offsets[n]):
+        if not flags[n] or n in folded:
+            continue
+        numel = int(np.prod(shapes[n], dtype=np.int64)) if len(shapes[n]) else 1
+        lo, hi = offsets[n], offsets[n] + (numel + 3) // 4 * 4
+        rows = [(c, min(c + CHUNK, hi)) for c in range(lo, hi, CHUNK)]
+        if tower_of(n) == "text":
+            out["text"] += rows
+            if text_done:
+                continue
+        out["main"] += rows
+    return out
 
 
 class TrainablePlan:
@@ -264,7 +293,7 @@
     _RUNTIME = ("_flat", "_flat_grad", "_flat16", "_offsets", "_ranges", "_layer_end", "_pmap", "_pool", "_trigger",
                 "_versions", "_w16", "_w16t", "_kp", "_kp_real", "_conv_pad", "_conv_gpad", "_cast_list", "_tjobs",
                 "_tjobs_bwd", "_adam_tiles_ok", "_wt_fresh", "_wt_event", "_aux_stream", "_mirror_fresh", "_mirror_versions", "_vdesc", "_tdesc", "_vblocks", "_tblocks",
-                "_side_streams", "_main_stream", "_pack_cache", "_cls_rows", "_sat", "_sat_poll", "_step_events", "grad_sync", "_w8", "_fp8_fresh", "_zero_table", "_zero_tables", "_adam_segs", "_first_touch", "_lease_batch", "_plist", "_plans", "_patch_pin", "_patch_off")
+                "_side_streams", "_main_stream", "_pack_cache", "_cls_rows", "_sat", "_sat_poll", "_step_events", "grad_sync", "_w8", "_fp8_fresh", "_zero_table", "_zero_tables", "_adam_segs", "_first_touch", "_gnorm", "_gnorm_request", "_gnorm_cache", "_lease_batch", "_plist", "_plans", "_patch_pin", "_patch_off")
 
     def __getstate__(self):
         state = dict(self.__dict__)
@@ -473,11 +502,34 @@
             check(lib().ce_zero_segments(ptr(self._flat_grad), ptr(table), table.shape[0], stream()), "ce_zero_segments")
 
     def zero_grad_first_touch(self):
+        acc = self.__dict__.pop("_gnorm_request", None)
+        self._gnorm = None
         if self._flat_grad is None or os.environ.get("CE_WGRAD_FIRST_TOUCH", "1") == "0":
             return self.zero_grad()
-        self._zero_segments(self._zero_table_for())
+        table = self._zero_table_for()
+        if acc is not None and table.shape[0]:
+            check(lib().ce_zero_segments_scalar(ptr(self._flat_grad), ptr(table), table.shape[0], ptr(acc), stream()),
+                  "ce_zero_segments_scalar")
+            self._gnorm = {"acc": acc, "folded": set(), "passes": {}, "text_done": False, "dirty": False}
+        else:
+            self._zero_segments(table)
         self._attach_grads_fast()
         self._first_touch = {"visual", "text"}
+
+    def _gnorm_chunks(self, piece: str, folded, text_done: bool):
+        flags = self._flags()
+        key = (flags, frozenset(folded), bool(text_done), self._flat_grad.data_ptr())
+        cache = self.__dict__.setdefault("_gnorm_cache", {})
+        hit = cache.get(key)
+        if hit is None:
+            named = list(self.named_parameters())
+            tables = gnorm_tables(self._offsets, {n: tuple(p.shape) for n, p in named}, {n: f for (n, _), f in zip(named, flags)},
+                                  folded, text_done)
+            if len(cache) >= 8:
+                cache.clear()
+            hit = cache[key] = {k: torch.tensor(v, dtype=torch.int64).reshape(-1, 2).to(self._flat_grad.device)
+                                for k, v in tables.items()}
+        return hit[piece]
 
     def _settle_first_touch(self):
         pending = getattr(self, "_first_touch", None)
@@ -491,6 +543,7 @@
 
     def zero_grad(self, set_to_none: bool = False):
         self._first_touch = set()
+        self._gnorm = None
         if self._flat_grad is not None and not set_to_none:
             self._flat_grad.zero_()
             self._attach_grads_fast()
diff --git a/clip_event_amd/optim.py b/clip_event_amd/optim.py
--- a/clip_event_amd/optim.py
+++ b/clip_event_amd/optim.py
@@ -13,6 +13,7 @@
 from ._lib import check, lib, ptr, stream
 
 MAX_GROUPS = 8
+_COUNT_NORM_ELEMENTS = os.environ.get("CE_GNORM_COUNT", "0") == "1"
 
 
 class OptimGroup(ctypes.Structure):
@@ -46,6 +47,8 @@
         self.step_count = 0
         self.sat_poll_every = int(os.environ.get("CE_SAT_POLL_EVERY", "16"))
         self.sumsq = None
+        self.norm_folded = False
+        self.norm_pass_elements = None
         self.ema = None
         self.ema_decay, self.ema_warmup, self.ema_updates = None, False, 0
         self._ema_of = None
@@ -120,6 +123,20 @@
     def _plain(self) -> bool:
         return len(self.param_groups) == 1 and not self.param_groups[0].get("decoupled_weight_decay") and all(self._flags_seen)
 
+    def _folded_norm(self, sumsq, s) -> bool:
+        m = self.model
+        gn = m.__dict__.get("_gnorm")
+        m._gnorm = None
+        self.norm_folded = bool(sumsq is not None and gn is not None and not gn["dirty"] and gn["acc"] is sumsq
+                                and getattr(m, "grad_sync", None) is None)
+        if not self.norm_folded:
+            return False
+        table = m._gnorm_chunks("main", gn["folded"], gn["text_done"])
+        if table.shape[0]:
+            check(lib().ce_sumsq_segments(ptr(m._flat_grad), ptr(table), table.shape[0], ptr(sumsq), s), "ce_sumsq_segments(rest)")
+        self.norm_pass_elements = int((table[:, 1] - table[:, 0]).sum()) if _COUNT_NORM_ELEMENTS else None
+        return True
+
     def _grouped_step(self, sumsq, s):
         m = self.model
         if getattr(getattr(m, "grad_sync", None), "plan", None) is not None:
@@ -133,7 +150,7 @@
         garr = (OptimGroup * len(self.param_groups))()
         for i, g in enumerate(self.param_groups):
             garr[i].lr, garr[i].weight_decay, garr[i].decoupled = float(g["lr"]), float(g["weight_decay"]), int(bool(g.get("decoupled_weight_decay")))
-        if sumsq is not None:
+        if sumsq is not None and not self._folded_norm(sumsq, s):
             sumsq.zero_()
             check(lib().ce_sumsq_segments(ptr(m._flat_grad), ptr(plan.chunks), plan.chunks.shape[0], ptr(sumsq), s),
                   "ce_sumsq_segments")
@@ -247,9 +264,14 @@
         self.model._flat_grad.zero_()
         self.model._attach_grads_fast()
 
-    def zero_grad_first_touch(self):
-        self._state()
-        self.model.zero_grad_first_touch()
+    def zero_grad_first_touch(self, fold_norm: bool = False):
+        self._state()
+        m = self.model
+        from . import distributed as D
+        if (fold_norm and self.max_norm is not None and os.environ.get("CE_GNORM_FOLD", "1") != "0"
+                and getattr(m, "grad_sync", None) is None and not D.active() and hasattr(m, "_gnorm_chunks")):
+            m._gnorm_request = self.sumsq
+        m.zero_grad_first_touch()
 
     def grad_norm(self) -> torch.Tensor:
         return self.sumsq.sqrt()
@@ -294,10 +316,11 @@
                                                          ptr(m._flat16[lo:hi]), hi - lo, *args, *ema, s), self._flat_op + suffix)
 
         if sharded:
+            m._gnorm = None
             D.sharded_update(plan, m._flat, sumsq, sum_squares, update)
             m.mark_operands_stale(mirror_fresh=False)
         else:
-            if sumsq is not None:
+            if sumsq is not None and not self._folded_norm(sumsq, s):
                 sumsq.zero_()
                 sum_squares(0, n)
             if getattr(m, "_adam_tiles_ok", False) and os.environ.get("CE_ADAM_TILES", "1") != "0":
diff --git a/include/clip_event_hip.h b/include/clip_event_hip.h
--- a/include/clip_event_hip.h
+++ b/include/clip_event_hip.h
@@ -43,6 +43,9 @@
 int ce_gemm_tn_grouped_ex(int count, const void* const* P, const long* ldp, const void* const* Q, const long* ldq, int M,
                           const int* Nn, const int* Kk, float* const* out, const long* ldo, int splits, int overwrite,
                           void* stream);
+int ce_gemm_tn_grouped_acc(int count, const void* const* P, const long* ldp, const void* const* Q, const long* ldq, int M,
+                           const int* Nn, const int* Kk, float* const* out, const long* ldo, int splits, int overwrite,
+                           float* sumsq_acc, void* stream);
 
 int ce_quant_rows_fp8(const void* x, long ldx, void* q, long ldq, float* scale, int M, int K, void* stream);
 typedef struct ce_quant_job {
@@ -187,6 +190,7 @@
 
 int ce_sumsq(const float* g, long n, float* out, void* stream);
 int ce_zero_segments(float* base, const long* table_device, int nchunks, void* stream);
+int ce_zero_segments_scalar(float* base, const long* table_device, int nchunks, float* scalar, void* stream);
 int ce_adam_step(float* p, const float* g, float* m, float* v, void* p_bf16, long n, const float* sumsq, float max_norm,
                  float lr, float beta1, float beta2, float eps, float weight_decay, int step, void* stream);
 typedef struct ce_transpose_job {
@@ -278,6 +282,7 @@
     int stream16;
     int wgrad_overwrite;
     const float* grad_scale;
+    float* gnorm_acc;
 } ce_tower_desc;
 
 size_t ce_tower_workspace_bytes(const ce_tower_desc* d, int batch);
@@ -292,6 +297,9 @@
                             void* workspace, void* dx, const int* sel_rows, const float* dx_sel, int layer_hi,
                             int layer_lo, void* stream);
 
+int ce_tower_backward_folds(const ce_tower_desc* d, int batch, int rows, int pruned, int layer_hi, int layer_lo,
+                            unsigned char* folded_out);
+
 int ce_ot_fwd(const float* txt, long tsb, long tsr, const float* img, long isb, long isr,
               const unsigned char* txt_pad, const unsigned char* img_pad, float* dist, float* T, float* txt_inv,
               float* img_inv, int B, int M, int N, int D, float beta, int iters, void* stream);
@@ -353,7 +361,7 @@
 enum {
     CE_PROF_GEMM_NT0 = 0,
     CE_PROF_GEMM_TN = 64, CE_PROF_ATTN_FWD = 65, CE_PROF_ATTN_BWD = 66, CE_PROF_LN_FWD = 67, CE_PROF_LN_BWD = 68,
-    CE_PROF_COLSUM = 69, CE_PROF_OTHER = 70, CE_PROF_GEMM_TN2 = 71 ,
+    CE_PROF_COLSUM = 69, CE_PROF_OTHER = 70, CE_PROF_GRAD_NORM = 70 , CE_PROF_GEMM_TN2 = 71 ,
     CE_PROF_GEMM_NT_QGELU = 72,
     CE_PROF_NCLASS = 80
 };
@@ -375,6 +383,8 @@
                  int tiles_n[CE_TN_MAX_GROUP], tiles_k[CE_TN_MAX_GROUP], tile_end[CE_TN_MAX_GROUP]; } ce_tn_plan;
 int ce_gemm_tn_plan(int count, const int* Nn, const int* Kk, int M, int splits, int overwrite,
                     const ce_tn_knobs* knobs, ce_tn_plan* out);
+int ce_gemm_tn_folds(int count, const int* Nn, const int* Kk, int M, int splits, int overwrite, const ce_tn_knobs* knobs,
+                     int* folded_out);
 int ce_tower_wgrad_cuts(int n_blocks, int width, int M, long extra_tiles, int force_group, int* sizes_out);
 void ce_gemm_nt_fp8_tune(int variant);
 
```

After: 21260 pairs/s (whole job), median of 6. Within noise of the previous version (+0.2%).
